# simonamtoft/downsampled-diffusion

Hardware: AMD Instinct MI355X
Metric: images/sec (T=1000 sampling), 256x256 dDDPM-x3 (higher is better)
Workload: dtype f32

## Files before the change

downsampled-diffusion_amd/csrc/conv_wino.hip:

```cpp
#include <atomic>
#include <cstdlib>
#include <type_traits>
#include <utility>

#include "cluster_sync.h"
#include "conv_common.h"
#include "pack_elems.h"

namespace ddk {

__device__ __attribute__((aligned(128))) float g_wino_zero[32];

struct WinoParams {
    const float* src0;
    const float* src1;
    const float* wu;
    const float* bias;
    const float* resid;
    float* out;
    int c0, c1, cin;
    int B, H, W, TH, TW;
    int N, tiles;
    int splits, chunks, chunks_per_split;
    long long slab_stride;
// ... 391 lines not shown
        };
        const float m2 = group_sum((sq4(keep[0][0]) + sq4(keep[0][1])) + (sq4(keep[1][0]) + sq4(keep[1][1])), red + 128);
        if (!CL) {
            if (tid < 16 && (cq & (qpg - 1)) == 0) p.gn_part[(long long)tile_m * p.groups + n0 / p.cpg + gl] = make_float2(mean, m2);
        } else {
            const int image = tile_m / p.cl_np;
            unsigned long long* rec = reinterpret_cast<unsigned long long*>(p.cl_rec) + ((long long)tile_m * gridDim.y + tile_n) * 16;
            unsigned* cnt = p.cl_cnt + ((long long)image * gridDim.y + tile_n) * 16;
            int* gave_up = reinterpret_cast<int*>(red + 256);
            if (tid == 0) *gave_up = 0;
            if (tid < 16 && (cq & (qpg - 1)) == 0) cl_store_stats(rec + gl, mean, m2);
            const int gn = n0 + (tid & 15) * 4;
            float4 ga, be, ts = make_float4(0.f, 0.f, 0.f, 0.f);
            auto load_affine = [&] {
                ga = *reinterpret_cast<const float4*>(p.gn_gamma + gn);
                be = *reinterpret_cast<const float4*>(p.gn_beta + gn);
                if (p.gn_temb) {
                    const int b_img = (int)((long long)t0 / ((long long)p.TH * p.TW));
                    const long long tr = p.gn_temb_rows ? p.gn_temb_rows[b_img] : b_img;
                    ts = *reinterpret_cast<const float4*>(p.gn_temb + tr * p.gn_temb_stride + gn);
                }
            };
            long long oo[2];
            float4 rs[2][2];
#pragma unroll
            for (int it = 0; it < 2; ++it) {
                const int item = tid + it * 512;
                const int t = item >> 5, a = (item >> 4) & 1;
                const int g = t0 + t;
                const unsigned tmp = fdiv_u((unsigned)g, p.dTW);
                const int tx = g - (int)tmp * p.TW;
                const unsigned bq = fdiv_u(tmp, p.dTH);
                const int ty = (int)tmp - (int)bq * p.TH;
                oo[it] = ((((long long)bq * p.H + 2 * ty + a) * p.W) + 2 * tx) * p.N + gn;
            }
            auto load_resid = [&] {
#pragma unroll
                for (int it = 0; it < 2; ++it) {
                    rs[it][0] = rs[it][1] = make_float4(0.f, 0.f, 0.f, 0.f);
                    if (p.resid) {
                        rs[it][0] = *reinterpret_cast<const float4*>(p.resid + oo[it]);
                        rs[it][1] = *reinterpret_cast<const float4*>(p.resid + oo[it] + p.N);
                    }
                }
            };
            if (wid != 0) { load_affine(); load_resid(); }
            if (wid == 0) {
                asm volatile("s_waitcnt vmcnt(0)" ::: "memory");
                if (lane == 0) __hip_atomic_fetch_add(cnt, 1u, __ATOMIC_RELAXED, __HIP_MEMORY_SCOPE_AGENT);
                load_affine();
                load_resid();
                if (lane == 0 && cl_wait_ge<4>(cnt, (unsigned)p.cl_np, p.cl_fail)) *gave_up = 1;
            }
            __syncthreads();
            const unsigned long long* r0 = reinterpret_cast<const unsigned long long*>(p.cl_rec) +
                                           ((long long)image * p.cl_np * gridDim.y + tile_n) * 16 + gl;
            const bool poisoned = *gave_up != 0;
            float rm[8], rq[8];
            cl_load_stats(r0, (long long)gridDim.y * 16, p.cl_np, rm, rq);
            if (tid == 0) cl_depart(cnt, cnt + 1, (unsigned)p.cl_np);
            const float2 st = cl_merge_stats(rm, rq, p.cl_np, 128.0f * (float)p.cpg, p.gn_eps, poisoned);
            const float gmean = st.x, rstd = st.y;
            auto fin = [&](float4 v) {
                return make_float4(mish_f((v.x - gmean) * rstd * ga.x + be.x) + ts.x, mish_f((v.y - gmean) * rstd * ga.y + be.y) + ts.y,
                                   mish_f((v.z - gmean) * rstd * ga.z + be.z) + ts.z, mish_f((v.w - gmean) * rstd * ga.w + be.w) + ts.w);
            };
#pragma unroll
            for (int it = 0; it < 2; ++it) {
                *reinterpret_cast<float4*>(p.out + oo[it]) = f4add(fin(keep[it][0]), rs[it][0]);
                *reinterpret_cast<float4*>(p.out + oo[it] + p.N) = f4add(fin(keep[it][1]), rs[it][1]);
            }
        }
    }
    if (DBG && tid == 0) {
        asm volatile("s_waitcnt vmcnt(0)" ::: "memory");
        const int wg = (blockIdx.x + gridDim.x * (blockIdx.y + gridDim.y * blockIdx.z)) & 1023;
        g_wino_stamps[wg * 8 + 6] = __builtin_amdgcn_s_memrealtime();
        g_wino_stamps[wg * 8 + 7] = 1;
    }
}

#include "conv_wino2_kernel.inc"
#include "conv_winoT_kernel.inc"

enum { WINO_V_OLD = 0, WINO_V_D = 1, WINO_V_F = 2 };
static int wino_variant(int B, int H, int W, int N) {
#ifdef DDK_TUNING
    if (const char* e = getenv("DDK_WINO_VARIANT")) {
        const int v = atoi(e);
        if (v == WINO_V_OLD || v == WINO_V_D || (v == WINO_V_F && N % 128 == 0)) return v;
    }
#endif
    const long long mt = ceil_div((long long)B * (H / 2) * (W / 2), WBT);
    return (N % 128 == 0 && mt * (N / 128) >= 224) ? WINO_V_F : WINO_V_D;
}
static int wino_nt(int variant) { return variant == WINO_V_F ? 128 : WBN; }
bool conv_wino_ok(int kind, int H, int W, int cin, int N) {
    return kind == DDK_CONV3X3_S1 && H >= 2 && W >= 2 && H % 2 == 0 && W % 2 == 0 && cin > 0 && cin % 32 == 0 && N % 64 == 0;
}

int conv_wino_splits(int B, int H, int W, int cin, int N) {
    const long long tiles = (long long)B * (H / 2) * (W / 2);
    const long long wgs = ceil_div(tiles, WBT) * (N / wino_nt(wino_variant(B, H, W, N)));
    const int chunks = cin / 32;
    int s = 1;
    while (wgs * s < 256 && s * 2 <= chunks) s *= 2;
    const int cps = (int)ceil_div(chunks, s);
    return (int)ceil_div(chunks, cps);
}

static int wino_stats_shape_parts(int B, int H, int W, int cin, int N, int groups) {
    if (!conv_wino_ok(DDK_CONV3X3_S1, H, W, cin, N) || groups <= 0 || N % groups) return 0;
    const int cpg = N / groups, tpi = (H / 2) * (W / 2), nt_w = wino_nt(wino_variant(B, H, W, N));
    if (cpg % 4 || nt_w % cpg || nt_w / cpg > 8 || tpi % WBT || tpi / WBT > 32) return 0;
    return tpi / WBT;
}
int conv_wino_stats_parts(int B, int H, int W, int cin, int N, int groups) {
    if (conv_wino_splits(B, H, W, cin, N) != 1) return 0;
    return wino_stats_shape_parts(B, H, W, cin, N, groups);
}

bool convT_wino_ok(int H, int W, int cin, int N) {
    return H >= 2 && W >= 2 && H % 2 == 0 && W % 2 == 0 && cin > 0 && cin % 32 == 0 && N > 0 && N % WT_NT == 0;
}
int convT_wino_splits(int B, int H, int W, int cin, int N) {
    const long long wgs = ceil_div((long long)B * (H / 2) * (W / 2), WBT) * (N / WT_NT) * 4;
    const int chunks = cin / 32;
    int s = 1;
    while (wgs * s < 256 && s * 2 <= chunks) s *= 2;
    const int cps = (int)ceil_div(chunks, s);
    return (int)ceil_div(chunks, cps);
}
int convT_wino_forward(const ddk_conv_args& a, int splits, hipStream_t st) {
    WinoParams p{};
    p.src0 = a.src0; p.wu = a.weight_wino; p.bias = a.bias; p.out = a.out;
    p.c0 = a.c0; p.c1 = 0; p.cin = a.c0;
    p.B = a.B; p.H = a.H; p.W = a.W; p.TH = a.H / 2; p.TW = a.W / 2;
    p.N = a.N; p.tiles = a.B * p.TH * p.TW;
    p.chunks = p.cin / 32;
    p.chunks_per_split = (int)ceil_div(p.chunks, splits);
    p.splits = (int)ceil_div(p.chunks, p.chunks_per_split);
    p.slab_stride = (long long)a.B * (2 * a.H) * (2 * a.W) * a.N;
    p.dTW = make_fastdiv_u((unsigned)p.TW);
    p.dTH = make_fastdiv_u((unsigned)p.TH);
    if (p.splits > 1) p.out = static_cast<float*>(a.workspace);
    dim3 grid((unsigned)ceil_div(p.tiles, WBT), (unsigned)(a.N / WT_NT), (unsigned)(4 * p.splits));
#ifdef DDK_TUNING
    if (getenv("DDK_WINO_STAMPS")) {
        hipLaunchKernelGGL(convT_wino_kernel<1>, grid, dim3(1024), WT_LDS_FL * sizeof(float), st, p);
        return check_launch("convT_wino_kernel<dbg>");
    }
#endif
    hipLaunchKernelGGL(convT_wino_kernel<0>, grid, dim3(1024), WT_LDS_FL * sizeof(float), st, p);
    return check_launch("convT_wino_kernel");
}

int conv_wino_init_device() {
    DDK_HIP(hipFuncSetAttribute(reinterpret_cast<const void*>(&convT_wino_kernel<0>), hipFuncAttributeMaxDynamicSharedMemorySize,
                                (int)(WT_LDS_FL * sizeof(float))));
#ifdef DDK_TUNING
    DDK_HIP(hipFuncSetAttribute(reinterpret_cast<const void*>(&convT_wino_kernel<1>), hipFuncAttributeMaxDynamicSharedMemorySize,
                                (int)(WT_LDS_FL * sizeof(float))));
#endif
    DDK_HIP(hipFuncSetAttribute(reinterpret_cast<const void*>(&conv3x3_wino_kernel<0>), hipFuncAttributeMaxDynamicSharedMemorySize,
                                (int)(W_LDS_FLOATS * sizeof(float))));
    DDK_HIP(hipFuncSetAttribute(reinterpret_cast<const void*>(&conv3x3_wino_kernel<0, true>), hipFuncAttributeMaxDynamicSharedMemorySize,
                                (int)(W_LDS_FLOATS * sizeof(float))));
    DDK_HIP(hipFuncSetAttribute(reinterpret_cast<const void*>(&conv3x3_wino2_kernel<2, 0, false>), hipFuncAttributeMaxDynamicSharedMemorySize,
                                (int)(W2<2>::LDS_FL * sizeof(float))));
    DDK_HIP(hipFuncSetAttribute(reinterpret_cast<const void*>(&conv3x3_wino2_kernel<2, 0, true>), hipFuncAttributeMaxDynamicSharedMemorySize,
                                (int)(W2<2>::LDS_FL * sizeof(float))));
    DDK_HIP(hipFuncSetAttribute(reinterpret_cast<const void*>(&conv3x3_wino2_kernel<4, 0, false>), hipFuncAttributeMaxDynamicSharedMemorySize,
                                (int)(W2<4>::LDS_FL * sizeof(float))));
    DDK_HIP(hipFuncSetAttribute(reinterpret_cast<const void*>(&conv3x3_wino2_kernel<4, 0, true>), hipFuncAttributeMaxDynamicSharedMemorySize,
                                (int)(W2<4>::LDS_FL * sizeof(float))));
#ifdef DDK_TUNING
#define W2_DBG_ATTR(P_, D_) DDK_HIP(hipFuncSetAttribute(reinterpret_cast<const void*>(&conv3x3_wino2_kernel<P_, D_, false>), \
                                                hipFuncAttributeMaxDynamicSharedMemorySize, (int)(W2<P_>::LDS_FL * sizeof(float))))
    W2_DBG_ATTR(2, 1); W2_DBG_ATTR(2, 7); W2_DBG_ATTR(2, 9); W2_DBG_ATTR(2, 15); W2_DBG_ATTR(2, 17);
    W2_DBG_ATTR(4, 1); W2_DBG_ATTR(4, 7); W2_DBG_ATTR(4, 9); W2_DBG_ATTR(4, 15); W2_DBG_ATTR(4, 17);
#undef W2_DBG_ATTR
    DDK_HIP(hipFuncSetAttribute(reinterpret_cast<const void*>(&conv3x3_wino_kernel<1>), hipFuncAttributeMaxDynamicSharedMemorySize, (int)(W_LDS_FLOATS * sizeof(float))));
    DDK_HIP(hipFuncSetAttribute(reinterpret_cast<const void*>(&conv3x3_wino_kernel<2>), hipFuncAttributeMaxDynamicSharedMemorySize, (int)(W_LDS_FLOATS * sizeof(float))));
    DDK_HIP(hipFuncSetAttribute(reinterpret_cast<const void*>(&conv3x3_wino_kernel<3>), hipFuncAttributeMaxDynamicSharedMemorySize, (int)(W_LDS_FLOATS * sizeof(float))));
    DDK_HIP(hipFuncSetAttribute(reinterpret_cast<const void*>(&conv3x3_wino_kernel<4>), hipFuncAttributeMaxDynamicSharedMemorySize, (int)(W_LDS_FLOATS * sizeof(float))));
#endif
    return DDK_OK;
}

int conv_wino_cluster_np(int B, int H, int W, int cin, int N, int groups) {
    const int np = conv_wino_stats_parts(B, H, W, cin, N, groups);
    if (np <= 0 || np > 8) return 0;
    const int nt_w = wino_nt(wino_variant(B, H, W, N));
    if (N / groups > 32 || nt_w % (N / groups)) return 0;
    if (nt_w / (N / groups) > 8) return 0;
    const long long mt = (long long)B * np, nt = N / nt_w;
    if ((mt * nt) % 8) return 0;
    const long long run = mt * nt / 8;
    const long long per_round = run < 32 ? run : 32;
    if (run % (np * nt) || per_round % (np * nt)) return 0;
    return np;
}
int conv_wino_cluster_split_np(int B, int H, int W, int cin, int N, int groups, int* splits_out) {
    if (!conv_wino_ok(DDK_CONV3X3_S1, H, W, cin, N)) return 0;
    const int splits = conv_wino_splits(B, H, W, cin, N);
    if (splits_out) *splits_out = splits;
    if (splits <= 1 || splits > 4) return 0;
    const int np = wino_stats_shape_parts(B, H, W, cin, N, groups);
    if (np <= 0 || np > 8) return 0;
    const int variant = wino_variant(B, H, W, N);
    if (variant != WINO_V_D) return 0;
    const int nt_w = wino_nt(variant);
    if (N / groups > 32 || nt_w % (N / groups) || nt_w / (N / groups) > 8) return 0;
    const long long mt = (long long)B * np, nt = N / nt_w;
    if (mt * nt * splits > 256) return 0;
    return np;
}
size_t conv_wino_cluster_pair_words(int B, int H, int W, int N) {
    return (size_t)ceil_div((long long)B * (H / 2) * (W / 2), WBT) * (size_t)(N / WBN) * 16;
}
size_t conv_wino_cluster_ws_floats(int B, int H, int W, int N) {
    const long long mt = (long long)B * (H / 2) * (W / 2) / WBT, nt = N / WBN;
    return (size_t)(mt * nt * 32 + (long long)B * nt * 16);
}

bool conv_wino_cluster_device_ok() {
    static std::atomic<int> cached[64];
    int dev = 0;
    if (hipGetDevice(&dev) != hipSuccess || dev < 0 || dev >= 64) return false;
    int v = cached[dev].load(std::memory_order_relaxed);
    if (v == 0) {
        int cus = 0, xccs = 0;
        bool ok = hipDeviceGetAttribute(&cus, hipDeviceAttributeMultiprocessorCount, dev) == hipSuccess && cus == 256;
        ok = ok && hipDeviceGetAttribute(&xccs, hipDeviceAttributeNumberOfXccs, dev) == hipSuccess && xccs == 8;
        ok = ok && !getenv("HSA_CU_MASK") && !getenv("ROC_GLOBAL_CU_MASK");
        (void)hipGetLastError();
        v = ok ? 1 : 2;
        cached[dev].store(v, std::memory_order_relaxed);
    }
    return v == 1;
// ... 60 lines not shown
    if (v == D_) {                                                                                                     \
        if (f) hipLaunchKernelGGL((conv3x3_wino2_kernel<2, D_, false>), grid2, dim3(768), lds, st, p);                 \
        else hipLaunchKernelGGL((conv3x3_wino2_kernel<4, D_, false>), grid2, dim3(768), lds, st, p);                   \
        return check_launch("conv3x3_wino2_kernel<dbg>");                                                              \
    }
            W2_DBG_LAUNCH(7) W2_DBG_LAUNCH(9) W2_DBG_LAUNCH(15) W2_DBG_LAUNCH(17)
#undef W2_DBG_LAUNCH
            if (f) hipLaunchKernelGGL((conv3x3_wino2_kernel<2, 1, false>), grid2, dim3(768), lds, st, p);
            else hipLaunchKernelGGL((conv3x3_wino2_kernel<4, 1, false>), grid2, dim3(768), lds, st, p);
            return check_launch("conv3x3_wino2_kernel<dbg>");
        }
#endif
        if (fuse) {
            if (f) hipLaunchKernelGGL((conv3x3_wino2_kernel<2, 0, true>), grid2, dim3(768), lds, st, p);
            else hipLaunchKernelGGL((conv3x3_wino2_kernel<4, 0, true>), grid2, dim3(768), lds, st, p);
            return check_launch("conv3x3_wino2_kernel<cluster>");
        }
        if (f) hipLaunchKernelGGL((conv3x3_wino2_kernel<2, 0, false>), grid2, dim3(768), lds, st, p);
        else hipLaunchKernelGGL((conv3x3_wino2_kernel<4, 0, false>), grid2, dim3(768), lds, st, p);
        return check_launch("conv3x3_wino2_kernel");
    }
    dim3 grid((unsigned)ceil_div(p.tiles, WBT), (unsigned)(a.N / WBN), (unsigned)p.splits);
#ifdef DDK_TUNING
    if (getenv("DDK_WINO_STAMPS")) {
        const int v = getenv("DDK_WINO_DEBUG") ? atoi(getenv("DDK_WINO_DEBUG")) : 1;
        if (v == 2) hipLaunchKernelGGL(conv3x3_wino_kernel<2>, grid, dim3(512), W_LDS_FLOATS * sizeof(float), st, p);
        else if (v == 3) hipLaunchKernelGGL(conv3x3_wino_kernel<3>, grid, dim3(512), W_LDS_FLOATS * sizeof(float), st, p);
        else if (v == 4) hipLaunchKernelGGL(conv3x3_wino_kernel<4>, grid, dim3(512), W_LDS_FLOATS * sizeof(float), st, p);
        else hipLaunchKernelGGL(conv3x3_wino_kernel<1>, grid, dim3(512), W_LDS_FLOATS * sizeof(float), st, p);
        return check_launch("conv3x3_wino_kernel<dbg>");
    }
#endif
    if (fuse) {
        hipLaunchKernelGGL((conv3x3_wino_kernel<0, true>), grid, dim3(512), W_LDS_FLOATS * sizeof(float), st, p);
        return check_launch("conv3x3_wino_kernel<cluster>");
    }
    hipLaunchKernelGGL(conv3x3_wino_kernel<0>, grid, dim3(512), W_LDS_FLOATS * sizeof(float), st, p);
    return check_launch("conv3x3_wino_kernel");
}

__global__ __launch_bounds__(256) void occupy_kernel(unsigned long long ticks, unsigned* sink) {
    extern __shared__ float occupy_lds[];
    occupy_lds[threadIdx.x] = (float)threadIdx.x;
    __syncthreads();
    const unsigned long long t_begin = __builtin_amdgcn_s_memrealtime();
    while (__builtin_amdgcn_s_memrealtime() - t_begin < ticks) __builtin_amdgcn_s_sleep(32);
    if (occupy_lds[(threadIdx.x + 1) & 255] < 0.f && sink) *sink = 1;
}

unsigned conv_wino_cluster_timeouts() { return cl_timeouts_read(); }

int cluster_fail_check(unsigned* word, hipStream_t st, const char* who, const char* tail) {
    unsigned v = 0;
    DDK_HIP(hipMemcpyAsync(&v, word, sizeof(v), hipMemcpyDeviceToHost, st));
    DDK_HIP(hipStreamSynchronize(st));
    if (v == 0) return DDK_OK;
    DDK_HIP(hipMemsetAsync(word, 0, sizeof(v), st));
    set_error("%s: %u workgroup(s) gave up waiting for their cluster%s", who, v, tail);
    return DDK_ERR_CLUSTER;
}

}

extern "C" int ddk_pack_conv_weight_wino(const float* w_oihw, float* dst, int O, int I, int i_pad, ddk_stream_t s) {
    using namespace ddk;
    DDK_REQUIRE(w_oihw && dst && O > 0 && I > 0 && i_pad >= I && i_pad % 32 == 0, "pack_conv_weight_wino: arguments (i_pad % 32 == 0)");
    const long long total = (long long)O * i_pad;
    DDK_REQUIRE(total < (1LL << 31), "pack_conv_weight_wino: 2^31 (n, c) pairs or more");
    const long long blocks = ceil_div(total, 256);
    hipLaunchKernelGGL(pack_conv_weight_wino_kernel<false>, dim3((unsigned)(blocks < 4096 ? blocks : 4096)), dim3(256), 0, as_stream(s), w_oihw,
                       dst, O, I, i_pad, total, 0, I);
    return check_launch("pack_conv_weight_wino_kernel");
}

extern "C" int ddk_pack_convT_weight_wino(const float* w_iohw, float* dst, int I, int O, int i_pad, ddk_stream_t s) {
    using namespace ddk;
    DDK_REQUIRE(w_iohw && dst && O > 0 && I > 0 && i_pad >= I && i_pad % 32 == 0, "pack_convT_weight_wino: arguments (i_pad % 32 == 0)");
    const long long total = (long long)O * i_pad;
    const long long blocks = ceil_div(total, 256);
    hipLaunchKernelGGL(pack_convT_weight_wino_kernel, dim3((unsigned)(blocks < 4096 ? blocks : 4096)), dim3(256), 0, as_stream(s), w_iohw, dst,
                       I, O, i_pad, total);
    return check_launch("pack_convT_weight_wino_kernel");
}
extern "C" int ddk_convT_wino_splits(int B, int H, int W, int cin, int N) {
    if (!ddk::convT_wino_ok(H, W, cin, N)) return 0;
    return ddk::convT_wino_splits(B, H, W, cin, N);
}

extern "C" int ddk_pack_conv_weight_wino_dgrad(const float* w_oihw, float* dst, int O, int I, int c_lo, int c_hi, int o_pad, ddk_stream_t s) {
    using namespace ddk;
    DDK_REQUIRE(w_oihw && dst && O > 0 && I > 0 && c_lo >= 0 && c_hi > c_lo && c_hi <= I && o_pad >= O && o_pad % 32 == 0,
                "pack_conv_weight_wino_dgrad: arguments (0 <= c_lo < c_hi <= I, o_pad % 32 == 0)");
    const long long total = (long long)(c_hi - c_lo) * o_pad;
    DDK_REQUIRE(total < (1LL << 31), "pack_conv_weight_wino_dgrad: 2^31 (n, c) pairs or more");
    const long long blocks = ceil_div(total, 256);
    hipLaunchKernelGGL(pack_conv_weight_wino_kernel<true>, dim3((unsigned)(blocks < 4096 ? blocks : 4096)), dim3(256), 0, as_stream(s), w_oihw,
                       dst, c_hi - c_lo, O, o_pad, total, c_lo, I);
    return check_launch("pack_conv_weight_wino_kernel<dgrad>");
}

#ifdef DDK_TUNING
extern "C" int ddk_debug_read_wino_timeline(unsigned long long* host_out) {
    if (hipDeviceSynchronize() != hipSuccess) return -2;
    return hipMemcpyFromSymbol(host_out, HIP_SYMBOL(ddk::g_wino_timeline), sizeof(unsigned long long) * 12 * 8 * 2) == hipSuccess ? 0 : -2;
}
extern "C" int ddk_debug_read_wino_stamps(unsigned long long* host_out) {
    if (hipDeviceSynchronize() != hipSuccess) return -2;
    if (hipMemcpyFromSymbol(host_out, HIP_SYMBOL(ddk::g_wino_stamps), sizeof(unsigned long long) * 8 * 1024) != hipSuccess) return -2;
    static unsigned long long zeros[8 * 1024];
    return hipMemcpyToSymbol(HIP_SYMBOL(ddk::g_wino_stamps), zeros, sizeof(zeros)) == hipSuccess ? 0 : -2;
}
#endif

extern "C" int ddk_conv_gn_partials(int B, int H, int W, int cin, int N, int groups) {
    return ddk::conv_wino_stats_parts(B, H, W, cin, N, groups);
}

extern "C" int ddk_conv_wino_splits(int B, int H, int W, int cin, int N) {
    if (!ddk::conv_wino_ok(DDK_CONV3X3_S1, H, W, cin, N)) return 0;
    return ddk::conv_wino_splits(B, H, W, cin, N);
}

extern "C" int ddk_conv3x3_gn_mish_cluster_ok(int B, int H, int W, int cin, int N, int groups) {
    if (!ddk::conv_wino_cluster_device_ok()) return 0;
    const int np = ddk::conv_wino_cluster_np(B, H, W, cin, N, groups);
    return np > 0 ? np : ddk::conv_wino_cluster_split_np(B, H, W, cin, N, groups, nullptr);
}
extern "C" size_t ddk_conv3x3_gn_mish_cluster_workspace_bytes(int B, int H, int W, int N) {
    if (B <= 0 || H <= 0 || W <= 0 || N <= 0 || N % ddk::WBN) return 0;
    return ((size_t)B * 8 * 16 + 16 + ddk::conv_wino_cluster_ws_floats(B, H, W, N)) * sizeof(float);
}
extern "C" size_t ddk_conv3x3_gn_mish_cluster_split_workspace_bytes(int B, int H, int W, int cin, int N, int groups) {
    int splits = 1;
    if (ddk::conv_wino_cluster_split_np(B, H, W, cin, N, groups, &splits) <= 0) return 0;
    return ddk_conv3x3_gn_mish_cluster_workspace_bytes(B, H, W, N) +
           (ddk::conv_wino_cluster_pair_words(B, H, W, N) + (size_t)(splits - 1) * B * H * W * N) * sizeof(float);
}
extern "C" int ddk_conv3x3_gn_mish_cluster_check(void* workspace, int B, ddk_stream_t s) {
    using namespace ddk;
    DDK_REQUIRE(workspace && B > 0, "conv3x3_gn_mish_cluster_check: arguments");
    return cluster_fail_check(cl_words(static_cast<float*>(workspace), B).fail, as_stream(s), "conv3x3_gn_mish_cluster",
                              "; the output is invalid (NaN tiles)");
}

extern "C" int ddk_debug_occupy(int workgroups, int lds_bytes, int microseconds, ddk_stream_t s) {
    using namespace ddk;
    DDK_REQUIRE(workgroups > 0 && workgroups <= 4096 && lds_bytes >= 1024 && lds_bytes <= 160 * 1024 && microseconds > 0 &&
                    microseconds <= 200000, "debug_occupy: 1..4096 workgroups, 1 KiB..160 KiB of LDS, at most 0.2 s");
    DDK_HIP(hipFuncSetAttribute(reinterpret_cast<const void*>(&occupy_kernel), hipFuncAttributeMaxDynamicSharedMemorySize, lds_bytes));
    hipLaunchKernelGGL(occupy_kernel, dim3((unsigned)workgroups), dim3(256), (size_t)lds_bytes, as_stream(s),
                       (unsigned long long)microseconds * 100ull, static_cast<unsigned*>(nullptr));
    return check_launch("occupy_kernel");
}

extern "C" int ddk_conv3x3_gn_mish_cluster(const float* src0, int c0, const float* src1, int c1, const float* weight_wino, const float* bias,
                                           const float* gamma, const float* beta, const float* temb, int temb_stride, const float* addend,
                                           float* out, int B, int H, int W, int N, int groups, float eps, void* workspace,
                                           size_t workspace_bytes, ddk_stream_t s) {
    using namespace ddk;
    DDK_REQUIRE(src0 && weight_wino && gamma && beta && out && workspace, "conv3x3_gn_mish_cluster: null pointer");
    DDK_REQUIRE(conv_wino_cluster_device_ok() && ddk_conv3x3_gn_mish_cluster_ok(B, H, W, c0 + c1, N, groups) > 0,
                "conv3x3_gn_mish_cluster: shape or device not eligible (ddk_conv3x3_gn_mish_cluster_ok)");
    const size_t plain_bytes = ddk_conv3x3_gn_mish_cluster_workspace_bytes(B, H, W, N);
    const size_t split_bytes = ddk_conv3x3_gn_mish_cluster_split_workspace_bytes(B, H, W, c0 + c1, N, groups);
    DDK_REQUIRE(workspace_bytes >= (split_bytes ? split_bytes : plain_bytes) && aligned16(workspace), "conv3x3_gn_mish_cluster: workspace");
    float* ws = static_cast<float*>(workspace);
// ... 23 lines not shown
```

downsampled-diffusion_amd/csrc/ddk_internal.h:

```cpp
#pragma once
#include <hip/hip_runtime.h>

#include <cstdarg>
#include <cstdint>
#include <cstdio>

#include "ddk.h"

#ifdef DDK_HOST_SANITIZE
#include "host_sanitize.h"
#endif

namespace ddk {

void set_error(const char* fmt, ...);

inline int fail_arg(const char* what) {
    set_error("bad argument: %s", what);
    return DDK_ERR_ARG;
}

inline int check_launch(const char* what) {
    hipError_t e = hipGetLastError();
    if (e != hipSuccess) {
// ... 51 lines not shown

__device__ __forceinline__ float wave_sum(float v) {
#pragma unroll
    for (int o = 32; o > 0; o >>= 1) v += __shfl_xor(v, o, 64);
    return v;
}

__device__ __forceinline__ float wave_max(float v) {
#pragma unroll
    for (int o = 32; o > 0; o >>= 1) v = fmaxf(v, __shfl_xor(v, o, 64));
    return v;
}

__device__ __forceinline__ float block_sum(float v, float* red) {
    v = wave_sum(v);
    const int lane = threadIdx.x & 63, wid = threadIdx.x >> 6, nw = blockDim.x >> 6;
    __syncthreads();
    if (lane == 0) red[wid] = v;
    __syncthreads();
    float t = (lane < nw) ? red[lane] : 0.0f;
    t = wave_sum(t);
    return t;
}

__device__ __forceinline__ float block_max(float v, float* red) {
    v = wave_max(v);
    const int lane = threadIdx.x & 63, wid = threadIdx.x >> 6, nw = blockDim.x >> 6;
    __syncthreads();
    if (lane == 0) red[wid] = v;
    __syncthreads();
    float t = (lane < nw) ? red[lane] : -INFINITY;
    t = wave_max(t);
    return t;
}

int ensure_device_init();
int conv_init_device();
int wgrad_init_device();

size_t conv_workspace_bytes(int kind, int B, int H, int W, int cin, int N);
struct ConvLnFold {
    const float* c1;
    const float* c2;
    float eps;
};
struct WinoGnFuse {
    const float* gamma;
    const float* beta;
    const float* temb;
    const long long* temb_rows;
    int temb_stride;
    float eps;
    int groups;
    float* records;
    unsigned* counters;
    unsigned* fail;
    unsigned* pairs = nullptr;
    const float* res_x = nullptr;
    const float* res_w = nullptr;
    const float* res_b = nullptr;
    int res_cin = 0, res_ld = 0;
};
bool conv_ln_fold_ok(int B, int H, int W, int cin, int N);
int conv_forward(const ddk_conv_args& a, hipStream_t st, const ConvLnFold* ln = nullptr, const WinoGnFuse* fuse = nullptr);
int conv_splits(int kind, int B, int H, int W, int cin, int N);
bool conv_wino_ok(int kind, int H, int W, int cin, int N);
int conv_wino_splits(int B, int H, int W, int cin, int N);
int conv_wino_forward(const ddk_conv_args& a, int splits, hipStream_t st, const WinoGnFuse* fuse = nullptr);
int conv_wino_cluster_np(int B, int H, int W, int cin, int N, int groups);
int conv_wino_cluster_split_np(int B, int H, int W, int cin, int N, int groups, int* splits_out);
size_t conv_wino_cluster_pair_words(int B, int H, int W, int N);
bool conv_wino_variant_new(int B, int H, int W, int N);
bool conv_wino_cluster_device_ok();
size_t conv_wino_cluster_ws_floats(int B, int H, int W, int N);
unsigned conv_wino_cluster_timeouts();
unsigned conv_first_cluster_timeouts();
unsigned level_chain_cluster_timeouts();
struct ClWords { unsigned* counters; unsigned* fail; };
inline ClWords cl_words(float* cl, int B) { return {reinterpret_cast<unsigned*>(cl), reinterpret_cast<unsigned*>(cl + (size_t)B * 8 * 16)}; }
int cluster_fail_check(unsigned* word, hipStream_t st, const char* who, const char* tail);
bool convT_wino_ok(int H, int W, int cin, int N);
int convT_wino_splits(int B, int H, int W, int cin, int N);
int convT_wino_forward(const ddk_conv_args& a, int splits, hipStream_t st);
int conv_wino_init_device();
int conv_wino_stats_parts(int B, int H, int W, int cin, int N, int groups);
bool conv_first_ok(int cin, int N, int H, int W, int groups);
int conv_first(const float* x, const float* wp, const float* bias, float* out, float* gn_partials, int B, int H, int W, int cin, int N,
               int groups, int64_t* counter, int64_t* t_cur, hipStream_t st);
int conv_first_init_device();
bool conv_first_gn_ok(int cin, int N, int H, int W, int groups);
size_t conv_first_gn_ws_floats(int B, int H, int W);
int conv_first_gn(const float* x, const float* wp, const float* bias, const float* gamma, const float* beta, const float* temb,
                  int temb_stride, const long long* temb_rows, float eps, float* out, int B, int H, int W, int cin, int N, int groups,
                  float* records, unsigned* counters, unsigned* fail, int64_t* counter, int64_t* t_cur, hipStream_t st);
bool conv1x1_sm_ok(long long M, int c0, int c1, int N);
int conv1x1_sm(const float* src0, int c0, const float* src1, int c1, const float* w, const float* bias, const float* resid, float* out,
               long long M, int N, const ConvLnFold* ln, hipStream_t st);
int conv1x1_sm_init_device();
bool conv1x1_stream_ok(long long M, int cin, int N);
int conv1x1_stream(const float* x, int cin, const float* w, const float* bias, const float* dmish_src, const float* resid, float* out,
                   float* mish_out, long long M, int N, int pre_mish, int post_mish, hipStream_t st);
bool conv1x1_ws_ok(long long M, int K, int N);
int conv1x1_ws(const float* x, const float* w, const float* bias, const float* resid, float* out, long long M, int N, const ConvLnFold* ln,
               hipStream_t st, int images = 0);
int conv1x1_ws_init_device();
struct AddendSlabs {
    int n = 1;
    long long stride = 0;
    const float* bias = nullptr;
};
bool conv_gn_local_ok(int H, int W, int cin, int c0, int N, int groups);
int conv_gn_local(const float* src0, int c0, const float* src1, int c1, const float* w, const float* bias, const float* gamma,
                  const float* beta, const float* temb, int temb_stride, const long long* temb_rows, const float* addend, float* out,
                  int B, int H, int W, int N, int groups, float eps, hipStream_t st, const AddendSlabs& as = AddendSlabs(),
                  const AddendSlabs& src_slabs = AddendSlabs());
int conv_gn_local_init_device();
bool conv_gn_wlocal_ok(int H, int W, int cin, int c0, int N, int groups);
int conv_gn_wlocal(const float* src0, int c0, const float* src1, int c1, const float* w, const float* bias, const float* gamma,
                   const float* beta, const float* temb, int temb_stride, const long long* temb_rows, const float* addend, float* out,
                   int B, int H, int W, int N, int groups, float eps, hipStream_t st, const AddendSlabs& as = AddendSlabs(),
                   const AddendSlabs& src_slabs = AddendSlabs());
double conv_flops(int kind, int B, int H, int W, int cin, int N);
size_t groupnorm_workspace_bytes(int B, int HW, int C, int groups);
int gn_train_nsplit(int HW, int cpg);
int gn_stats_partials(const float* x, float* part, int B, int HW, int C, int groups, int ns, hipStream_t st);
int groupnorm_mish(const float* x, const float* gamma, const float* beta, const float* temb, int temb_stride,
                   const float* addend, float* out, int B, int HW, int C, int groups, float eps, void* ws, size_t ws_bytes,
                   hipStream_t st, const long long* temb_rows = nullptr);
int groupnorm_mish_ex(const float* x, int nslab, long long slab_stride, const float* cbias, const float* gamma,
                      const float* beta, const float* temb, int temb_stride, const float* addend, float* out, int B, int HW, int C,
                      int groups, float eps, void* ws, size_t ws_bytes, hipStream_t st, const long long* temb_rows = nullptr);
int groupnorm_mish_parts(const float* x, const float* part, int np, const float* gamma, const float* beta, const float* temb,
                         int temb_stride, const float* addend, float* out, int B, int HW, int C, int groups, float eps, hipStream_t st,
                         const long long* temb_rows = nullptr, const float* rc_x = nullptr, const float* rc_w = nullptr,
                         const float* rc_b = nullptr, int rc_cin = 0, int rc_ld = 0);
int chan_layernorm(const float* x, const float* g, const float* b, float* out, long long M, int C, float eps, hipStream_t st);
int groupnorm_mish_generic(const float* x, const float* gamma, const float* beta, const float* temb, int temb_stride, const float* addend,
                           float* out, int B, int HW, int CP, int C, int groups, float eps, hipStream_t st, const long long* temb_rows = nullptr);
int chan_layernorm_generic(const float* x, const float* g, const float* b, float* out, long long M, int CP, int C, float eps, hipStream_t st);
int unary(int op, const float* x, float* out, long long n, hipStream_t st);
int add(const float* a, const float* b, float* out, long long n, hipStream_t st);
int avgpool2(const float* x, float* out, int B, int H, int W, int C, hipStream_t st);
int upsample_nearest2(const float* x, float* out, int B, int H, int W, int C, hipStream_t st);
size_t linattn_context_workspace_bytes(int B, int HW, int heads);
int linattn_context(const float* qkv, float* ctx, int B, int HW, int heads, void* workspace, size_t workspace_bytes, hipStream_t st,
                    bool kv_only = false);
bool attn_fold_ok(int C, int heads);
bool attn_kvctx_ok(int B, int HW, int C, int heads);
size_t attn_kvctx_workspace_bytes(int B, int HW);
int attn_kvctx(const float* x, const float* w_kv, const float* c1, const float* c2, float ln_eps, float* ctx, int B, int HW, void* workspace,
               size_t workspace_bytes, hipStream_t st);
size_t attn_fold_out_floats(int B);
int attn_fold(const float* ctx, const float* wqg, const float* c1q, const float* c2q, const float* wout, const float* bout, float* A,
              float* a1, float* a2, int B, int C, int heads, hipStream_t st);
int linattn_apply(const float* qkv, const float* ctx, float* out, int B, int HW, int heads, hipStream_t st);
int linattn_fused_small(const float* qkv, float* ctx, float* out, int B, int HW, int heads, hipStream_t st);
bool linattn_small_qkv_ok(int HW, int C);
int linattn_small_qkv_init_device();
int qkv_operand_pack(const float* lnw, float* wop, int heads, int cp, hipStream_t st);
int linattn_small_qkv(const float* x, const float* wop, const float* c1, const float* c2, float ln_eps, float* ctx, float* out, int B, int HW,
                      int C, int heads, hipStream_t st);
int time_mlp(const int64_t* t, const float* freqs, const float* w1t, const float* b1, const float* w2t, const float* b2,
             float* act, float* raw, int B, int dim, hipStream_t st);
int time_proj(const float* act, const float* wt, const float* bias, float* out, int B, int dim, int n_out, hipStream_t st);
int conv1x1_small_n(const float* x, const float* w, const float* bias, float* out, long long M, int C, int n_out, hipStream_t st);
struct InpaintOps {
// ... 75 lines not shown
```

downsampled-diffusion_amd/csrc/unet_plan.hip:

```cpp
#include <algorithm>
#include <mutex>
#include <string>
#include <vector>

#include "ddk_internal.h"
#include "level_chain.h"

namespace ddk {

constexpr int HEADS = 4;
constexpr int HIDDEN = HEADS * 32;
constexpr int GROUPS = 8;
constexpr float GN_EPS = 1e-5f, LN_EPS = 1e-5f;

static inline int pad32(int c) { return (c + 31) / 32 * 32; }

enum PackKind { PK_COPY = 0, PK_CONV = 1, PK_CONVT = 2, PK_LINEAR_T = 3, PK_WINO = 4, PK_LOCAL = 5, PK_WLOCAL = 6, PK_FIRST = 7, PK_CONVT_WINO = 8,
                PK_ROWS = 9 , PK_LOCAL1 = 10 ,
                PK_CONVT_LOCAL = 11  };

struct Slot {
    std::string name;
    long long numel;
    int kind;
    size_t off;
    int O, I, KH, KW, i_pad, ld, col0;
    int split = 0, split_pad = 0;
    int attn = -1;
};

struct ConvW {
    size_t w = 0, b = 0;
    bool has_bias = false;
    int cin = 0, cin_pad = 0, cout = 0;
    size_t wu = 0;
    bool has_wu = false;
    size_t wl = 0;
    bool has_wl = false;
    size_t wwl = 0;
    bool has_wwl = false;
    size_t wf = 0;
    bool has_wf = false;
    size_t wl1 = 0;
    bool has_wl1 = false;
    size_t wtl = 0;
    bool has_wtl = false;
};
struct NormW { size_t g = 0, b = 0; int c_real = 0; };
struct ResW {
    int ci = 0, ci_pad = 0, co = 0, temb_off = 0, ci_real = 0, co_real = 0;
    ConvW c1, c2, res;
    NormW n1, n2;
    bool has_res = false;
};
struct AttnW {
    int c = 0, c_real = 0;
    NormW ln;
    ConvW qkv, out;
    size_t qkv_lnw = 0, ln_c1 = 0, ln_c2 = 0;
    size_t qkv_op = 0;
};

}

using namespace ddk;

struct ChainKey {
    StepKind kind;
    const void* bufs[12];
    const void* ws;
    const void* noise;
    int B, H, W, t_start, device;
    unsigned long long pack_epoch;
    bool operator==(const ChainKey& o) const {
        for (int i = 0; i < 12; ++i)
            if (bufs[i] != o.bufs[i]) return false;
        return kind == o.kind && ws == o.ws && noise == o.noise && B == o.B && H == o.H && W == o.W && t_start == o.t_start &&
               device == o.device && pack_epoch == o.pack_epoch;
    }
};
struct SamplerGraph {
    ChainKey key;
    hipGraph_t graph = nullptr;
    hipGraphExec_t exec = nullptr;
    hipGraph_t graph_multi = nullptr;
    hipGraphExec_t exec_multi = nullptr;
    hipEvent_t done = nullptr;
    unsigned long long last_use = 0;
};
constexpr int SAMPLER_MULTI = 16;

struct ddk_unet {
    std::mutex mu;
    std::vector<SamplerGraph> graphs;
    unsigned long long use_clock = 0;
    unsigned long long pack_epoch = 0;
    struct {
        const void* ws = nullptr;
        int t_start = -1, B = 0, H = 0, W = 0;
        unsigned long long pack_epoch = 0;
        std::vector<int64_t> map;
    } table;
    ddk_unet_config cfg;
    int cluster_gn = 1;
    int cluster_limit = 1 << 30;
    int cluster_np_max = 8;
    bool cluster_split = true;
    bool attn_kvctx = true;
    bool fold_down_reduce = false;
    bool first_gn = true;
    int level_chain = 9;
    int level_chain_max_batch = 32;
    int attn_fold_min_hw = 256;
    bool attn_fold = true;
    bool generic = false;
    std::vector<int> dimp;
    std::vector<Slot> slots;
    size_t packed_floats = 0;
    int L = 0;
    std::vector<int> dims;
    int time_dim = 0, temb_total = 0;
    size_t freqs = 0, w1t = 0, b1 = 0, w2t = 0, b2 = 0, temb_wt = 0, temb_bias = 0;
    std::vector<ResW> down_res, up_res;
    std::vector<AttnW> down_attn, up_attn;
    std::vector<ConvW> down_conv, up_conv;
    ResW mid1, mid2;
    AttnW mid_attn;
    ConvW final_conv;
    NormW final_norm;
    size_t final_w = 0, final_b = 0;

    size_t alloc(size_t n) {
        const size_t o = packed_floats;
        packed_floats += (n + 3) / 4 * 4;
        return o;
    }
    size_t add_copy(const std::string& name, long long n) {
        const size_t o = alloc((size_t)n);
        slots.push_back(Slot{name, n, PK_COPY, o, 0, 0, 0, 0, 0, 0, 0});
        return o;
    }
    void add_copy_at(const std::string& name, long long n, size_t off) {
        slots.push_back(Slot{name, n, PK_COPY, off, 0, 0, 0, 0, 0, 0, 0});
    }
    ConvW add_conv(const std::string& prefix, int cout, int cin, int k, bool bias, bool gn_follows = false, int split = 0, bool local = false) {
        ConvW c;
        c.cin = cin; c.cin_pad = split > 0 ? pad32(split) + pad32(cin - split) : pad32(cin); c.cout = cout;
        const int cout_rows = pad32(cout);
        c.w = alloc((size_t)cout_rows * k * k * c.cin_pad);
        Slot sl{prefix + "weight", (long long)cout * cin * k * k, PK_CONV, c.w, cout, cin, k, k, c.cin_pad, 0, 0};
        if (split > 0 && c.cin_pad != cin) { sl.split = split; sl.split_pad = pad32(split); }
        slots.push_back(sl);
        c.has_bias = bias;
        if (bias) {
            c.b = alloc((size_t)cout_rows);
            slots.push_back(Slot{prefix + "bias", cout, PK_COPY, c.b, 0, 0, 0, 0, 0, 0, 0});
        }
        if (generic) return c;
        if (k == 1 && bias && cout % 32 == 0 && c.cin_pad == cin && cin % 32 == 0) {
            c.wl1 = alloc((size_t)cout * c.cin_pad);
            c.has_wl1 = true;
            slots.push_back(Slot{prefix + "weight", (long long)cout * cin, PK_LOCAL1, c.wl1, cout, cin, 1, 1, c.cin_pad, 0, 0});
        }
        if (k == 3 && cout % 64 == 0) {
            c.wu = alloc((size_t)16 * cout * c.cin_pad);
            c.has_wu = true;
            slots.push_back(Slot{prefix + "weight", (long long)cout * cin * k * k, PK_WINO, c.wu, cout, cin, k, k, c.cin_pad, 0, 0});
        }
        if (k == 3 && (gn_follows || local) && cout % 32 == 0) {
            c.wl = alloc((size_t)9 * cout * c.cin_pad);
            c.has_wl = true;
            slots.push_back(Slot{prefix + "weight", (long long)cout * cin * k * k, PK_LOCAL, c.wl, cout, cin, k, k, c.cin_pad, 0, 0});
            if (gn_follows && (c.cin_pad <= 320 || c.cin_pad == 512)) {
                c.wwl = alloc((size_t)16 * cout * c.cin_pad);
                c.has_wwl = true;
                slots.push_back(Slot{prefix + "weight", (long long)cout * cin * k * k, PK_WLOCAL, c.wwl, cout, cin, k, k, c.cin_pad, 0, 0});
            }
        }
        return c;
    }
    ConvW add_convT(const std::string& prefix, int ch, bool local = false) {
        ConvW c;
        c.cin = ch; c.cin_pad = pad32(ch); c.cout = ch;
        c.w = alloc((size_t)16 * pad32(ch) * pad32(ch));
        slots.push_back(Slot{prefix + "weight", (long long)16 * ch * ch, PK_CONVT, c.w, ch, ch, 4, 4, pad32(ch), 0, 0});
        c.has_bias = true;
        c.b = alloc((size_t)pad32(ch));
        slots.push_back(Slot{prefix + "bias", ch, PK_COPY, c.b, 0, 0, 0, 0, 0, 0, 0});
        if (local && ch % 32 == 0 && !generic) {
            c.wtl = alloc((size_t)16 * ch * ch);
            c.has_wtl = true;
            slots.push_back(Slot{prefix + "weight", (long long)16 * ch * ch, PK_CONVT_LOCAL, c.wtl, ch, ch, 4, 4, ch, 0, 0});
// ... 38 lines not shown
        a.c = generic ? pad32(c) : c;
        a.c_real = c;
        const size_t s0 = slots.size();
        a.qkv = add_conv(p + "fn.fn.to_qkv.", 3 * HIDDEN, c, 1, false);
        const size_t s1 = slots.size();
        a.out = add_conv(p + "fn.fn.to_out.", c, HIDDEN, 1, true);
        const size_t s2 = slots.size();
        a.ln = add_norm(p + "fn.norm.g", p + "fn.norm.b", c);
        for (size_t i = s0; i < s1; ++i) slots[i].attn = n_attn;
        for (size_t i = s2; i < slots.size(); ++i) slots[i].attn = n_attn;
        a.qkv_lnw = alloc((size_t)3 * HIDDEN * pad32(c));
        a.ln_c1 = alloc((size_t)3 * HIDDEN);
        a.ln_c2 = alloc((size_t)3 * HIDDEN);
        a.qkv_op = alloc((size_t)3 * HIDDEN * pad32(c));
        attn_all.push_back(a);
        ++n_attn;
        return a;
    }
};

static int total_temb(const ddk_unet& u) {
    int tot = 0;
    for (int l = 0; l < u.L; ++l) tot += 2 * u.dims[l + 1];
    tot += 2 * u.dims[u.L];
    for (int i = 0; i < u.L - 1; ++i) tot += 2 * u.dims[u.L - 1 - i];
    return tot;
}

extern "C" ddk_unet* ddk_unet_create(const ddk_unet_config* cfg) {
    if (!cfg || cfg->n_levels < 1 || cfg->n_levels > 8 || cfg->in_ch < 1 || cfg->chan < 8 || cfg->chan % 8 ||
        cfg->chan > 512) {
        set_error("unet_create: need 1 <= n_levels <= 8, in_ch >= 1, unet_chan a multiple of 8 in [8, 512]");
        return nullptr;
    }
    for (int i = 0; i < cfg->n_levels; ++i)
        if (cfg->mults[i] < 1) { set_error("unet_create: unet_dims entries must be >= 1"); return nullptr; }
    if (cfg->mults[0] != 1) {
        set_error("unet_create: unet_dims[0] must be 1 (the reference's final Block(dim, dim) meets dim * unet_dims[0] channels "
                  "otherwise and raises, unet.py:69-72)");
        return nullptr;
    }
    {
        int ndev = 0;
        if (hipGetDeviceCount(&ndev) == hipSuccess && ndev > 0 && ensure_device_init() != DDK_OK) return nullptr;
        (void)hipGetLastError();
    }
    ddk_unet* u = new ddk_unet();
    u->cfg = *cfg;
    u->L = cfg->n_levels;
    u->generic = cfg->chan % 32 != 0;
    for (int i = 0; i < cfg->n_levels; ++i)
        if (cfg->chan * cfg->mults[i] > 512) { set_error("unet_create: level widths above 512 channels are not supported"); delete u; return nullptr; }
    u->dims.push_back(cfg->in_ch);
    for (int i = 0; i < u->L; ++i) u->dims.push_back(cfg->chan * cfg->mults[i]);
    for (int d : u->dims) u->dimp.push_back(u->generic ? pad32(d) : d);
    u->time_dim = cfg->chan;
    u->temb_total = total_temb(*u);
    const int td = u->time_dim;

    u->freqs = u->add_copy("@sinusoidal_freqs", td / 2);
    u->w1t = u->alloc((size_t)td * 4 * td);
    u->slots.push_back(Slot{"time_mlp.1.weight", (long long)4 * td * td, PK_LINEAR_T, u->w1t, 4 * td, td, 0, 0, 0, 4 * td, 0});
    u->b1 = u->add_copy("time_mlp.1.bias", 4 * td);
    u->w2t = u->alloc((size_t)4 * td * td);
    u->slots.push_back(Slot{"time_mlp.3.weight", (long long)4 * td * td, PK_LINEAR_T, u->w2t, td, 4 * td, 0, 0, 0, td, 0});
    u->b2 = u->add_copy("time_mlp.3.bias", td);
    u->temb_wt = u->alloc((size_t)td * u->temb_total);
    u->temb_bias = u->alloc((size_t)u->temb_total);

    int cur = 0;
    for (int l = 0; l < u->L; ++l) {
        const std::string p = "downs." + std::to_string(l) + ".";
        const int ci = u->dims[l], co = u->dims[l + 1];
        u->down_res.push_back(u->add_res(p + "0.", ci, co, cur));
        if (l == 0 && ci <= 8 && co <= 256 && !u->generic) {
            ConvW& c1 = u->down_res[0].c1;
            const int K2 = (9 * ci + 1) / 2;
            c1.wf = u->alloc((size_t)(co / 32) * K2 * 64);
            c1.has_wf = true;
            u->slots.push_back(Slot{p + "0.block1.block.0.weight", (long long)co * ci * 9, PK_FIRST, c1.wf, co, ci, 3, 3, 0, 0, 0});
        }
        u->down_res.push_back(u->add_res(p + "1.", co, co, cur));
        u->down_attn.push_back(u->add_attn(p + "2.", co));
        if (l < u->L - 1) u->down_conv.push_back(u->add_conv(p + "3.conv.", co, co, 3, true, false, 0, l == u->L - 2));
    }
    const int mid = u->dims[u->L];
    u->mid1 = u->add_res("mid_block1.", mid, mid, cur);
    u->mid_attn = u->add_attn("mid_attn.", mid);
    u->mid2 = u->add_res("mid_block2.", mid, mid, cur);
    for (int i = 0; i < u->L - 1; ++i) {
        const std::string p = "ups." + std::to_string(i) + ".";
        const int din = u->dims[u->L - 1 - i], dout = u->dims[u->L - i];
        u->up_res.push_back(u->add_res(p + "0.", 2 * dout, din, cur, dout));
        u->up_res.push_back(u->add_res(p + "1.", din, din, cur));
        u->up_attn.push_back(u->add_attn(p + "2.", din));
        u->up_conv.push_back(u->add_convT(p + "3.conv.", din, i == 0));
    }
    u->final_conv = u->add_conv("final_conv.0.block.0.", cfg->chan, cfg->chan, 3, true, true);
    u->final_norm = u->add_norm("final_conv.0.block.1.weight", "final_conv.0.block.1.bias", cfg->chan);
    if (u->generic) {
        u->final_w = u->alloc((size_t)cfg->in_ch * pad32(cfg->chan));
        u->slots.push_back(Slot{"final_conv.1.weight", (long long)cfg->in_ch * cfg->chan, PK_ROWS, u->final_w, cfg->in_ch, cfg->chan, 0, 0, 0,
                                pad32(cfg->chan), 0});
    } else {
        u->final_w = u->add_copy("final_conv.1.weight", (long long)cfg->in_ch * cfg->chan);
    }
    u->final_b = u->add_copy("final_conv.1.bias", cfg->in_ch);
    if (cur != u->temb_total) {
        set_error("unet_create: internal temb accounting mismatch");
        delete u;
        return nullptr;
    }
    return u;
}

static void drop_graphs(ddk_unet* u) {
    for (SamplerGraph& g : u->graphs) {
        if (g.exec) (void)hipGraphExecDestroy(g.exec);
        if (g.graph) (void)hipGraphDestroy(g.graph);
        if (g.exec_multi) (void)hipGraphExecDestroy(g.exec_multi);
        if (g.graph_multi) (void)hipGraphDestroy(g.graph_multi);
        if (g.done) (void)hipEventDestroy(g.done);
    }
    u->graphs.clear();
    u->table.ws = nullptr;
}

extern "C" void ddk_unet_destroy(ddk_unet* u) {
    if (!u) return;
    if (!u->graphs.empty()) (void)hipDeviceSynchronize();
    drop_graphs(u);
    delete u;
}

extern "C" int ddk_sampler_invalidate(ddk_unet* u) {
    DDK_REQUIRE(u, "sampler_invalidate: null plan");
    std::lock_guard<std::mutex> lock(u->mu);
    if (!u->graphs.empty()) DDK_HIP(hipDeviceSynchronize());
    drop_graphs(u);
    return DDK_OK;
}
static void destroy_entry(SamplerGraph& g) {
    if (g.done) { (void)hipEventSynchronize(g.done); (void)hipEventDestroy(g.done); }
    if (g.exec) (void)hipGraphExecDestroy(g.exec);
    if (g.graph) (void)hipGraphDestroy(g.graph);
    if (g.exec_multi) (void)hipGraphExecDestroy(g.exec_multi);
    if (g.graph_multi) (void)hipGraphDestroy(g.graph_multi);
}

extern "C" int ddk_sampler_release_workspace(ddk_unet* u, const void* workspace) {
    DDK_REQUIRE(u && workspace, "sampler_release_workspace: arguments");
    std::lock_guard<std::mutex> lock(u->mu);
    for (size_t i = 0; i < u->graphs.size();) {
        if (u->graphs[i].key.ws == workspace) {
            destroy_entry(u->graphs[i]);
            u->graphs.erase(u->graphs.begin() + (long)i);
        } else {
            ++i;
        }
    }
    if (u->table.ws == workspace) u->table.ws = nullptr;
    return DDK_OK;
}

extern "C" int ddk_unet_set_option(ddk_unet* u, int option, int value) {
    DDK_REQUIRE(u, "unet_set_option: null plan");
    static const struct {
        int option;
        bool drops_graphs;
        void (*set)(ddk_unet&, int);
    } options[] = {
        {DDK_OPT_CLUSTER_GROUPNORM, true, [](ddk_unet& p, int v) { p.cluster_gn = v < 0 ? 0 : v > 2 ? 2 : v; }},
        {DDK_OPT_ATTENTION_FOLD, true, [](ddk_unet& p, int v) { p.attn_fold = v != 0; }},
        {DDK_OPT_ATTENTION_KV_CONTEXT, true, [](ddk_unet& p, int v) { p.attn_kvctx = v != 0; }},
        {DDK_OPT_FIRST_GROUPNORM, true, [](ddk_unet& p, int v) { p.first_gn = v != 0; }},
        {DDK_OPT_LEVEL_CHAIN, true, [](ddk_unet& p, int v) {
             p.level_chain = v == 1 ? 9 : v == 2 ? 1 : v == 3 ? 15 : v == 4 ? 6 : v == 8 ? 2 : v == 16 ? 4 : v != 0 ? 9 : 0;
         }},
        {DDK_OPT_FOLD_DOWNSAMPLE_REDUCE, true, [](ddk_unet& p, int v) { p.fold_down_reduce = v != 0; }},
        {10, true, [](ddk_unet& p, int v) { p.level_chain_max_batch = v; }},
        {9, true, [](ddk_unet& p, int v) { p.attn_fold_min_hw = v; }},
        {2, false, [](ddk_unet& p, int v) { p.cluster_limit = v; }},
        {4, true, [](ddk_unet& p, int v) { p.cluster_np_max = v; }},
        {11, true, [](ddk_unet& p, int v) { p.cluster_split = v != 0; }},
    };
    for (const auto& o : options) {
        if (o.option != option) continue;
        std::lock_guard<std::mutex> lock(u->mu);
        if (o.drops_graphs) {
            if (!u->graphs.empty()) DDK_HIP(hipDeviceSynchronize());
            drop_graphs(u);
        }
        o.set(*u, value);
        return DDK_OK;
    }
    return fail_arg("unet_set_option: unknown option");
}
extern "C" unsigned ddk_debug_cluster_timeouts(void) {
    unsigned sum = 0;
    for (unsigned v : {ddk::conv_wino_cluster_timeouts(), ddk::conv_first_cluster_timeouts(), ddk::level_chain_cluster_timeouts()}) {
        if (v == ~0u) return ~0u;
        sum += v;
    }
    return sum;
}
extern "C" int ddk_unet_num_slots(const ddk_unet* u) { return u ? (int)u->slots.size() : 0; }
extern "C" const char* ddk_unet_slot_name(const ddk_unet* u, int slot) {
    return (u && slot >= 0 && slot < (int)u->slots.size()) ? u->slots[slot].name.c_str() : nullptr;
}
extern "C" long long ddk_unet_slot_numel(const ddk_unet* u, int slot) {
    return (u && slot >= 0 && slot < (int)u->slots.size()) ? u->slots[slot].numel : -1;
}
extern "C" size_t ddk_unet_packed_bytes(const ddk_unet* u) { return u ? u->packed_floats * sizeof(float) : 0; }

__global__ __launch_bounds__(64) void ln_fold_kernel(const float* __restrict__ w, const float* __restrict__ g, const float* __restrict__ b,
                                                     float* __restrict__ wg, float* __restrict__ c1, float* __restrict__ c2, int C, int cp) {
    const int n = blockIdx.x;
    float s1 = 0.f, s2 = 0.f;
    for (int c = threadIdx.x; c < cp; c += 64) {
        const float wv = w[(long long)n * cp + c];
        const float gv = c < C ? g[c] : 0.f, bv = c < C ? b[c] : 0.f;
        wg[(long long)n * cp + c] = wv * gv;
        s1 += wv * gv;
        s2 += wv * bv;
    }
    s1 = wave_sum(s1);
    s2 = wave_sum(s2);
    if (threadIdx.x == 0) { c1[n] = s1; c2[n] = s2; }
}

static int fold_attn(const AttnW& a, float* P, hipStream_t st) {
    hipLaunchKernelGGL(ln_fold_kernel, dim3(3 * HIDDEN), dim3(64), 0, st, P + a.qkv.w, P + a.ln.g, P + a.ln.b, P + a.qkv_lnw, P + a.ln_c1,
                       P + a.ln_c2, a.c, pad32(a.c));
    DDK_TRY(check_launch("ln_fold_kernel"));
    return qkv_operand_pack(P + a.qkv_lnw, P + a.qkv_op, HEADS, pad32(a.c), st);
}

static void weights_changed(const ddk_unet* u) {
    ddk_unet* m = const_cast<ddk_unet*>(u);
    std::lock_guard<std::mutex> lock(m->mu);
    ++m->pack_epoch;
}

extern "C" int ddk_unet_finalize_pack(const ddk_unet* u, void* packed, ddk_stream_t s) {
    DDK_REQUIRE(u && packed, "unet_finalize_pack: arguments");
    weights_changed(u);
    for (const AttnW& a : u->attn_all) DDK_TRY(fold_attn(a, static_cast<float*>(packed), as_stream(s)));
    return DDK_OK;
}

extern "C" int ddk_unet_pack_slot(const ddk_unet* u, int slot, const float* canonical, void* packed, ddk_stream_t s) {
    DDK_REQUIRE(u && canonical && packed && slot >= 0 && slot < (int)u->slots.size(), "unet_pack_slot: arguments");
    const Slot& sl = u->slots[slot];
    float* dst = static_cast<float*>(packed) + sl.off;
    weights_changed(u);
    int rc;
    switch (sl.kind) {
        case PK_COPY:
            DDK_HIP(hipMemcpyAsync(dst, canonical, (size_t)sl.numel * sizeof(float), hipMemcpyDeviceToDevice, as_stream(s)));
            rc = DDK_OK;
            break;
        case PK_CONV:
            rc = sl.split > 0 ? ddk_pack_conv_weight_split(canonical, dst, sl.O, sl.I, sl.KH, sl.KW, sl.i_pad, sl.split, sl.split_pad, s)
                              : ddk_pack_conv_weight(canonical, dst, sl.O, sl.I, sl.KH, sl.KW, sl.i_pad, s);
            break;
        case PK_CONVT: rc = sl.i_pad == sl.I ? ddk_pack_convT_weight(canonical, dst, sl.I, sl.O, s)
                                             : ddk_pack_convT_weight_padded(canonical, dst, sl.I, sl.O, sl.i_pad, s); break;
        case PK_ROWS:
            DDK_HIP(hipMemcpy2DAsync(dst, (size_t)sl.ld * sizeof(float), canonical, (size_t)sl.I * sizeof(float), (size_t)sl.I * sizeof(float),
                                     (size_t)sl.O, hipMemcpyDeviceToDevice, as_stream(s)));
            rc = DDK_OK;
            break;
        case PK_LINEAR_T: rc = ddk_pack_linear_T(canonical, dst, sl.O, sl.I, sl.ld, sl.col0, s); break;
        case PK_WINO: rc = ddk_pack_conv_weight_wino(canonical, dst, sl.O, sl.I, sl.i_pad, s); break;
        case PK_LOCAL: rc = ddk_pack_conv_weight_local(canonical, dst, sl.O, sl.I, sl.i_pad, s); break;
        case PK_LOCAL1: rc = ddk_pack_conv1x1_weight_local(canonical, dst, sl.O, sl.I, sl.i_pad, s); break;
        case PK_CONVT_LOCAL: rc = ddk_pack_convT_weight_local(canonical, dst, sl.I, sl.O, s); break;
        case PK_WLOCAL: rc = ddk_pack_conv_weight_wino_local(canonical, dst, sl.O, sl.I, sl.i_pad, s); break;
        case PK_FIRST: rc = ddk_pack_conv_weight_first(canonical, dst, sl.O, sl.I, s); break;
        case PK_CONVT_WINO: rc = ddk_pack_convT_weight_wino(canonical, dst, sl.I, sl.O, sl.i_pad, s); break;
        default: return fail_arg("unet_pack_slot: slot kind");
    }
    DDK_TRY(rc);
    if (sl.attn >= 0) DDK_TRY(fold_attn(u->attn_all[sl.attn], static_cast<float*>(packed), as_stream(s)));
    return DDK_OK;
}

namespace ddk {

struct Layout {
    size_t act = 0;
    size_t qkv = 0, o = 0, ctx = 0, splitk = 0, gn_ws = 0, cl = 0, chain = 0;
    std::vector<size_t> skip;
    size_t xpad = 0, temb = 0, tact = 0;
    size_t off_A = 0, off_B = 0, off_C = 0, off_raw = 0, off_a1 = 0, off_res = 0, off_xn = 0, off_qkv = 0, off_o = 0, off_ctx = 0,
           off_splitk = 0, off_gn = 0, off_xpad = 0, off_temb = 0, off_tact = 0, off_cl = 0, off_chain = 0;
    std::vector<size_t> off_skip;
    size_t total = 0;
};

static size_t al4(size_t n) { return (n + 3) / 4 * 4; }

static void upd(size_t& m, size_t v) { if (v > m) m = v; }

static bool convT_wino_use(int B, int H, int W, int cin, int N) {
    return convT_wino_ok(H, W, cin, N) && convT_wino_splits(B, H, W, cin, N) <= 2;
}
static bool use_wino(const ConvW& cw, int H, int W, int cin, int N) {
    return cw.has_wu && conv_wino_ok(DDK_CONV3X3_S1, H, W, cin, N);
}
static int conv3_splits(const ConvW& cw, int B, int H, int W, int cin, int N) {
    return use_wino(cw, H, W, cin, N) ? conv_wino_splits(B, H, W, cin, N) : conv_splits(DDK_CONV3X3_S1, B, H, W, cin, N);
}
static size_t conv3_ws_floats(const ConvW& cw, int B, int H, int W, int cin, int N) {
    if (!use_wino(cw, H, W, cin, N)) return conv_workspace_bytes(DDK_CONV3X3_S1, B, H, W, cin, N) / 4;
    const int s = conv_wino_splits(B, H, W, cin, N);
    return s > 1 ? (size_t)s * B * H * W * N : 0;
}

constexpr size_t CL_PAIR_WORDS = 128 * 16;
static size_t cl_counter_floats(int B) { return (size_t)B * 8 * 16 + 16 + (size_t)B * 64 + CL_PAIR_WORDS; }
static size_t cl_chain_offset(int B) { return (size_t)B * 8 * 16 + 16; }
static size_t cl_pair_offset(int B) { return (size_t)B * 8 * 16 + 16 + (size_t)B * 64; }
constexpr int CHAIN_BUFS = 18;
constexpr int CHAIN8_BUFS = 5;

static void res_sizes(const ResW& r, int B, int H, int W, Layout& ly) {
    const size_t M = (size_t)B * H * W;
    upd(ly.act, M * r.co);
    upd(ly.splitk, conv3_ws_floats(r.c1, B, H, W, r.ci_pad, r.co));
    upd(ly.splitk, conv3_ws_floats(r.c2, B, H, W, r.co, r.co));
    if (r.has_res) upd(ly.splitk, conv_workspace_bytes(DDK_CONV1X1, B, H, W, r.ci_pad, r.co) / 4);
    upd(ly.gn_ws, groupnorm_workspace_bytes(B, H * W, r.co, GROUPS) / 4);
    upd(ly.gn_ws, (size_t)2 * GROUPS * (M / 128 + 1));
    upd(ly.cl, cl_counter_floats(B) + conv_wino_cluster_ws_floats(B, H, W, r.co));
    if (H * W % 128 == 0 && H * W / 128 <= 8) upd(ly.cl, cl_counter_floats(B) + conv_first_gn_ws_floats(B, H, W));
}

static void attn_sizes(const AttnW& a, int B, int H, int W, Layout& ly) {
    const size_t M = (size_t)B * H * W;
    upd(ly.act, M * a.c);
    upd(ly.qkv, M * 3 * HIDDEN);
    upd(ly.o, M * HIDDEN);
    upd(ly.ctx, (size_t)B * HEADS * 32 * 32);
    upd(ly.splitk, linattn_context_workspace_bytes(B, H * W, HEADS) / 4);
    if (attn_kvctx_ok(B, H * W, a.c, HEADS)) upd(ly.splitk, attn_kvctx_workspace_bytes(B, H * W) / 4);
    upd(ly.splitk, conv_workspace_bytes(DDK_CONV1X1, B, H, W, a.c, 3 * HIDDEN) / 4);
    upd(ly.splitk, conv_workspace_bytes(DDK_CONV1X1, B, H, W, HIDDEN, a.c) / 4);
}

static bool chain_plain(const ResW& r, bool wino) {
    return r.ci == 256 && r.co == 256 && !r.has_res && r.c1.has_bias && r.c2.has_bias && (wino ? r.c1.has_wwl && r.c2.has_wwl : r.c1.has_wl && r.c2.has_wl);
}
static bool chain_att(const AttnW& a) { return a.c == 256 && a.out.has_wl1 && a.out.has_bias; }
static bool chain_cat(const ResW& r, bool wino) {
    return r.ci == 512 && r.ci_pad == 512 && r.co == 256 && r.has_res && r.res.has_wl1 && r.res.has_bias && r.c1.cin_pad == 512 && r.c1.has_bias &&
           r.c2.has_bias && (wino ? r.c1.has_wwl && r.c2.has_wwl : r.c1.has_wl && r.c2.has_wl);
}
static bool level_chain_shape_ok(const ddk_unet& u, int H0, int W0) {
    if (u.generic || u.L < 2) return false;
    const int sh = u.L - 1;
    if ((H0 >> sh) != 4 || (W0 >> sh) != 4 || (H0 & ((1 << sh) - 1)) || (W0 & ((1 << sh) - 1))) return false;
    if (u.dimp[u.L] != 256 || u.dimp[u.L - 1] != 256 || GROUPS != 8) return false;
    return chain_plain(u.down_res[2 * sh], false) && chain_plain(u.down_res[2 * sh + 1], false) && chain_plain(u.mid1, false) &&
           chain_plain(u.mid2, false) && chain_plain(u.up_res[1], false) && chain_att(u.down_attn[sh]) && chain_att(u.mid_attn) &&
           chain_att(u.up_attn[0]) && chain_cat(u.up_res[0], false);
}
static bool level8_chain_shape_ok(const ddk_unet& u, int H0, int W0) {
    if (u.generic || u.L < 3) return false;
    const int sh = u.L - 2;
    if ((H0 >> sh) != 8 || (W0 >> sh) != 8 || (H0 & ((1 << sh) - 1)) || (W0 & ((1 << sh) - 1))) return false;
    if (u.dimp[sh + 1] != 256 || u.dimp[sh] != 256 || u.dimp[sh + 2] != 256 || GROUPS != 8) return false;
    return chain_plain(u.down_res[2 * sh], true) && chain_plain(u.down_res[2 * sh + 1], true) && chain_att(u.down_attn[sh]) &&
           chain_cat(u.up_res[2], true) && chain_plain(u.up_res[3], true) && chain_att(u.up_attn[1]);
}

static Layout make_layout(const ddk_unet& u, int B, int H0, int W0) {
    Layout ly;
    int H = H0, W = W0;
    ly.skip.resize(u.L);
    for (int l = 0; l < u.L; ++l) {
        res_sizes(u.down_res[2 * l], B, H, W, ly);
        res_sizes(u.down_res[2 * l + 1], B, H, W, ly);
        attn_sizes(u.down_attn[l], B, H, W, ly);
        ly.skip[l] = al4((size_t)B * H * W * u.dimp[l + 1]);
        if (l < u.L - 1) {
            upd(ly.splitk, conv_workspace_bytes(DDK_CONV3X3_S2, B, H, W, u.dimp[l + 1], u.dimp[l + 1]) / 4);
            H /= 2; W /= 2;
            upd(ly.act, (size_t)B * H * W * u.dimp[l + 1]);
// ... 459 lines not shown
    Ctx c{u, P, ws, ly, B, st, temb_table ? temb_table : temb, temb_table ? reinterpret_cast<const long long*>(t) : nullptr};
    if (!fast0) { c.x_first = x; c.x_padded = xpad; }
    c.allow_cluster = allow_cluster;
    float* bufA = ws + ly.off_A;
    float* bufB = ws + ly.off_B;
    float* bufC = ws + ly.off_C;
    float* raw = ws + ly.off_raw;
    float* a1 = ws + ly.off_a1;
    float* gnp = ws + ly.off_gn;

    int H = H0, W = W0;
    const float* cur = xpad;
    int cur_c = pad32(u.cfg.in_ch);
    AddendSlabs cur_ss;
    const bool first_fused = fast0 && c.allow_cluster && u.first_gn && conv_wino_cluster_device_ok() &&
                             conv_first_gn_ok(u.down_res[0].ci, u.down_res[0].co, H0, W0, GROUPS) && u.cluster_limit > 0;
    int64_t* dec_counter = (first_fused && step) ? step->state : nullptr;
    const bool chained = level_chain_use(c, H0, W0);
    const bool chain_edges = chained && (u.level_chain & 8) && u.L >= 2 && u.down_conv[u.L - 2].has_wl && u.down_conv[u.L - 2].has_bias &&
                             u.up_conv[0].has_wtl && u.up_conv[0].cin == 256 && u.down_conv[u.L - 2].cin == 256;
    const bool chained8 = level8_chain_use(c, H0, W0, 2);
    const bool chained8u = level8_chain_use(c, H0, W0, 4);
    for (int l = 0; l < u.L; ++l) {
        float* skip = ws + ly.off_skip[l];
        const int co = u.dimp[l + 1];
        if (chained && l == u.L - 1) {
            DDK_TRY(run_level_chain(c, 0, cur, skip, bufB, chain_edges ? ws + ly.off_skip[l - 1] : nullptr, chain_edges ? bufA : nullptr));
            cur_c = co;
            break;
        }
        const bool level_chained = chained8 && l == u.L - 2 && cur_ss.n == 1;
        if (level_chained) {
            DDK_TRY(run_level_chain(c, 1, cur, skip, nullptr));
        } else if (l == 0 && fast0) {
            const ResW& r = u.down_res[0];
            if (first_fused) {
                float* cl = ws + ly.off_cl;
                const ClWords w = cl_words(cl, B);
                DDK_TRY(conv_first_gn(x, P + r.c1.wf, r.c1.has_bias ? P + r.c1.b : nullptr, P + r.n1.g, P + r.n1.b, c.temb + r.temb_off,
                                      u.temb_total, c.temb_rows, GN_EPS, a1, B, H, W, r.ci, r.co, GROUPS, cl + cl_counter_floats(B),
                                      w.counters, w.fail,
                                      step ? step->state : nullptr, step ? t : nullptr, st));
            } else {
                DDK_TRY(conv_first(x, P + r.c1.wf, r.c1.has_bias ? P + r.c1.b : nullptr, raw, gnp, B, H, W, r.ci, r.co, GROUPS,
                                   step ? step->state : nullptr, step ? t : nullptr, st));
                DDK_TRY(groupnorm_mish_parts(raw, gnp, H * W / 128, P + r.n1.g, P + r.n1.b, c.temb + r.temb_off, u.temb_total, nullptr, a1, B,
                                             H * W, r.co, GROUPS, GN_EPS, st, c.temb_rows));
            }
            ddk_conv_args a{};
            a.kind = DDK_CONV3X3_S1;
            a.src0 = a1; a.c0 = r.co;
            a.weight = P + r.c2.w;
            a.weight_wino = P + r.c2.wu;
            a.bias = r.c2.has_bias ? P + r.c2.b : nullptr;
            a.B = B; a.H = H; a.W = W; a.N = r.co;
            const int cl_np = c.allow_cluster && conv_wino_cluster_device_ok() && r.ci <= 8 ? conv_wino_cluster_np(B, H, W, r.co, r.co, GROUPS) : 0;
            if (cl_np > 0 && cl_np <= u.cluster_np_max && conv_wino_variant_new(B, H, W, r.co) && c.n_cluster++ < u.cluster_limit) {
                a.out = bufB;
                float* cl = ws + ly.off_cl;
                const ClWords w = cl_words(cl, B);
                WinoGnFuse f{P + r.n2.g, P + r.n2.b, nullptr, nullptr, u.temb_total, GN_EPS, GROUPS, cl + cl_counter_floats(B), w.counters, w.fail};
                f.res_x = x; f.res_w = P + r.res.w; f.res_b = r.res.has_bias ? P + r.res.b : nullptr; f.res_cin = r.ci; f.res_ld = r.res.cin_pad;
                DDK_TRY(conv_forward(a, st, nullptr, &f));
            } else {
                a.out = raw;
                a.gn_partials = gnp;
                a.gn_groups = GROUPS;
                DDK_TRY(conv_forward(a, st));
                DDK_TRY(groupnorm_mish_parts(raw, gnp, conv_wino_stats_parts(B, H, W, r.co, r.co, GROUPS), P + r.n2.g, P + r.n2.b, nullptr,
                                             u.temb_total, nullptr, bufB, B, H * W, r.co, GROUPS, GN_EPS, st, nullptr, x, P + r.res.w,
                                             r.res.has_bias ? P + r.res.b : nullptr, r.ci, r.res.cin_pad));
            }
        } else {
            DDK_TRY(run_res(c, u.down_res[2 * l], cur, cur_c, nullptr, 0, bufB, H, W, cur_ss));
            cur_ss = AddendSlabs();
        }
        if (!level_chained) {
            DDK_TRY(run_res(c, u.down_res[2 * l + 1], bufB, co, nullptr, 0, bufC, H, W));
            DDK_TRY(run_attn(c, u.down_attn[l], bufC, skip, H, W));
        }
        if (l < u.L - 1 && chain_edges && l + 1 == u.L - 1) {
            H /= 2; W /= 2;
            cur = skip;
        } else if (l < u.L - 1) {
            const int s2 = conv_splits(DDK_CONV3X3_S2, B, H, W, co, co);
            if (u.fold_down_reduce && s2 > 1 && !(chained && l + 1 == u.L - 1) && !(chained8 && l + 1 == u.L - 2) &&
                res_takes_slab_source(u, u.down_res[2 * l + 2], B, H / 2, W / 2, co)) {
                ddk_conv_args a{};
                a.kind = DDK_CONV3X3_S2;
                a.src0 = skip; a.c0 = co;
                a.weight = P + u.down_conv[l].w;
                a.out = bufA;
                a.B = B; a.H = H; a.W = W; a.N = co;
                a.defer_reduce = 1;
                a.workspace = ws + ly.off_splitk;
                a.workspace_bytes = ly.splitk * sizeof(float);
                DDK_TRY(conv_forward(a, st));
                cur_ss.n = s2;
                cur_ss.stride = (long long)B * (H / 2) * (W / 2) * co;
                cur_ss.bias = u.down_conv[l].has_bias ? P + u.down_conv[l].b : nullptr;
                H /= 2; W /= 2;
                cur = ws + ly.off_splitk;
            } else {
                DDK_TRY(run_conv(c, DDK_CONV3X3_S2, u.down_conv[l], skip, co, nullptr, 0, nullptr, bufA, H, W, co));
                H /= 2; W /= 2;
                cur = bufA;
            }
        } else {
            cur = skip;
        }
        cur_c = co;
    }
    if (!chained) {
        DDK_TRY(run_res(c, u.mid1, cur, cur_c, nullptr, 0, bufB, H, W));
        DDK_TRY(run_attn(c, u.mid_attn, bufB, bufC, H, W));
        DDK_TRY(run_res(c, u.mid2, bufC, cur_c, nullptr, 0, bufA, H, W));
        cur = bufA;
    }
    for (int i = 0; i < u.L - 1; ++i) {
        const int lvl = u.L - 1 - i;
        const float* skip = ws + ly.off_skip[lvl];
        const int dout = u.dimp[lvl + 1], din = u.dimp[lvl];
        if (chained8u && i == 1) {
            DDK_TRY(run_level_chain(c, 2, cur, const_cast<float*>(skip), bufB));
        } else if (!(chained && i == 0)) {
            DDK_TRY(run_res(c, u.up_res[2 * i], cur, cur_c, skip, dout, bufB, H, W));
            DDK_TRY(run_res(c, u.up_res[2 * i + 1], bufB, din, nullptr, 0, bufC, H, W));
            DDK_TRY(run_attn(c, u.up_attn[i], bufC, bufB, H, W));
        }
        if (!(chain_edges && i == 0))
            DDK_TRY(run_conv(c, DDK_CONVT4X4_S2, u.up_conv[i], bufB, din, nullptr, 0, nullptr, bufA, H, W, din));
        H *= 2; W *= 2;
        cur = bufA;
        cur_c = din;
    }
    const int chan = u.generic ? pad32(u.cfg.chan) : u.cfg.chan, n_out = u.cfg.in_ch;
    StepRule plain{};
    plain.kind = StepKind::Eps;
    plain.eps_out = out;
    const StepRule& rule = step ? step->rule : plain;
    ChainHooks hooks{};
    if (step) {
        hooks.chain_state = step->state;
        hooks.dec_counter = dec_counter;
    }
    const int npf = fused_tail_parts(u, B, H, W, cur_c, rule.kind);
    if (npf > 0 && (!step || step->per == (long long)H * W * n_out)) {
        ddk_conv_args a{};
        a.kind = DDK_CONV3X3_S1;
        a.src0 = cur; a.c0 = cur_c;
        a.weight = P + u.final_conv.w;
        a.weight_wino = P + u.final_conv.wu;
        a.bias = u.final_conv.has_bias ? P + u.final_conv.b : nullptr;
        a.out = raw;
        a.B = B; a.H = H; a.W = W; a.N = chan;
        a.gn_partials = gnp;
        a.gn_groups = GROUPS;
        DDK_TRY(conv_forward(a, st));
        const TailIn in{raw, gnp, npf, P + u.final_norm.g, P + u.final_norm.b, GN_EPS, P + u.final_w, P + u.final_b, n_out, B, H * W, chan, GROUPS};
        return final_tail(in, rule, t, hooks, st);
    }
    DDK_TRY(run_conv_gn(c, u.final_conv, cur, cur_c, nullptr, 0, raw, u.final_norm, nullptr, nullptr, a1, H, W, chan));
    float* eps_hat = step ? step->eps_hat : out;
    DDK_TRY(conv1x1_small_n(a1, P + u.final_w, P + u.final_b, eps_hat, (long long)B * H * W, chan, n_out, st));
    return step ? p_update(rule, eps_hat, t, B, step->per, hooks, st) : DDK_OK;
}
// ... 32 lines not shown
        set_error("unet_forward: workspace too small (%zu < %zu)", workspace_bytes, ly.total * sizeof(float));
        return DDK_ERR_WORKSPACE;
    }
    float* ws = static_cast<float*>(workspace);
    DDK_TRY(ensure_device_init());
    DDK_HIP(hipMemsetAsync(ws + ly.off_cl, 0, cl_counter_floats(B) * sizeof(float), as_stream(s)));
    return forward_core(*u, static_cast<const float*>(packed), x, const_cast<int64_t*>(t), out, B, H, W, ws, ly, as_stream(s),
                        u->cluster_gn >= 2);
}

extern "C" int ddk_unet_cluster_check(const ddk_unet* u, void* workspace, int B, int H, int W, ddk_stream_t s) {
    DDK_TRY(check_shape(u, B, H, W));
    DDK_REQUIRE(workspace, "unet_cluster_check: null workspace");
    const Layout ly = make_layout(*u, B, H, W);
    return cluster_fail_check(cl_words(static_cast<float*>(workspace) + ly.off_cl, B).fail, as_stream(s), "in-launch GroupNorm",
                              " (the GPU is shared, masked or partitioned); results on this workspace are invalid -- rerun with "
                              "DDK_OPT_CLUSTER_GROUPNORM = 0");
}

extern "C" double ddk_unet_flops(const ddk_unet* u, int B, int H0, int W0) {
    if (check_shape(u, B, H0, W0) != DDK_OK) return 0;
    double f = 0;
    auto res = [&](const ResW& r, int H, int W) {
        f += conv_flops(DDK_CONV3X3_S1, B, H, W, r.ci_real, r.co_real) + conv_flops(DDK_CONV3X3_S1, B, H, W, r.co_real, r.co_real);
        if (r.has_res) f += conv_flops(DDK_CONV1X1, B, H, W, r.ci_real, r.co_real);
        f += 2.0 * B * u->time_dim * r.co_real;
    };
    auto attn = [&](const AttnW& a, int H, int W) {
        f += conv_flops(DDK_CONV1X1, B, H, W, a.c_real, 3 * HIDDEN) + conv_flops(DDK_CONV1X1, B, H, W, HIDDEN, a.c_real);
        f += 2.0 * 2.0 * B * HEADS * 32.0 * 32.0 * H * W;
    };
    int H = H0, W = W0;
    f += 2.0 * B * (u->time_dim * 4.0 * u->time_dim) * 2;
    for (int l = 0; l < u->L; ++l) {
        res(u->down_res[2 * l], H, W); res(u->down_res[2 * l + 1], H, W); attn(u->down_attn[l], H, W);
        if (l < u->L - 1) { f += conv_flops(DDK_CONV3X3_S2, B, H, W, u->dims[l + 1], u->dims[l + 1]); H /= 2; W /= 2; }
    }
    res(u->mid1, H, W); attn(u->mid_attn, H, W); res(u->mid2, H, W);
    for (int i = 0; i < u->L - 1; ++i) {
        res(u->up_res[2 * i], H, W); res(u->up_res[2 * i + 1], H, W); attn(u->up_attn[i], H, W);
        f += conv_flops(DDK_CONVT4X4_S2, B, H, W, u->up_conv[i].cin, u->up_conv[i].cout);
        H *= 2; W *= 2;
    }
    f += conv_flops(DDK_CONV3X3_S1, B, H, W, u->cfg.chan, u->cfg.chan) + conv_flops(DDK_CONV1X1, B, H, W, u->cfg.chan, u->cfg.in_ch);
    return f;
}

extern "C" double ddk_unet_flops_executed(const ddk_unet* u, int B, int H0, int W0) {
    if (check_shape(u, B, H0, W0) != DDK_OK) return 0;
    double f = 0;
    auto conv3 = [&](const ConvW& cw, int H, int W, int c0, int c1, int N, bool gn) {
        const int cin = c0 + c1;
        if (gn && cw.has_wl && (H * W == 16 || (H * W == 4 && B % 4 == 0)) && conv_gn_local_ok(H, W, cin, c0, N, GROUPS))
            return 2.0 * B * H * W * 9.0 * cin * N;
        if (gn && cw.has_wwl && H * W == 64 && conv_gn_wlocal_ok(H, W, cin, c0, N, GROUPS)) return 2.0 * B * (H * W / 4) * 16.0 * cin * N;
        if (use_wino(cw, H, W, cin, N)) return 2.0 * (double)(ceil_div((long long)B * (H / 2) * (W / 2), 32) * 32) * 16.0 * cin * N;
        return 2.0 * B * H * W * 9.0 * cin * N;
    };
    auto res = [&](const ResW& r, int H, int W, int c0, int c1, bool fast) {
        if (fast) {
            f += 2.0 * B * H * W * (2.0 * ((9 * r.ci + 1) / 2)) * r.co;
            f += 2.0 * B * H * W * (double)r.ci * r.co;
        } else {
            f += conv3(r.c1, H, W, c0, c1, r.co, true);
            if (r.has_res) f += conv_flops(DDK_CONV1X1, B, H, W, c0 + c1, r.co);
        }
        f += conv3(r.c2, H, W, r.co, 0, r.co, true);
    };
    auto attn = [&](const AttnW& a, int H, int W) {
        if (attn_fold_eligible(*u, a, B, H, W)) {
            f += conv_flops(DDK_CONV1X1, B, H, W, a.c, 2 * HIDDEN) + 2.0 * B * HEADS * 32.0 * 32.0 * H * W;
            f += 2.0 * B * (4.0 * HIDDEN * 32.0 * a.c + (double)a.c * HIDDEN * a.c) + conv_flops(DDK_CONV1X1, B, H, W, a.c, a.c);
            return;
        }
        f += conv_flops(DDK_CONV1X1, B, H, W, a.c, 3 * HIDDEN) + conv_flops(DDK_CONV1X1, B, H, W, HIDDEN, a.c);
        f += 2.0 * 2.0 * B * HEADS * 32.0 * 32.0 * H * W;
    };
    int H = H0, W = W0, cur_c = pad32(u->cfg.in_ch);
    for (int l = 0; l < u->L; ++l) {
        const int co = u->dims[l + 1];
        res(u->down_res[2 * l], H, W, cur_c, 0, l == 0 && first_fast(*u, B, H, W));
        res(u->down_res[2 * l + 1], H, W, co, 0, false);
        attn(u->down_attn[l], H, W);
        if (l < u->L - 1) { f += conv_flops(DDK_CONV3X3_S2, B, H, W, co, co); H /= 2; W /= 2; }
        cur_c = co;
    }
    res(u->mid1, H, W, cur_c, 0, false); attn(u->mid_attn, H, W); res(u->mid2, H, W, cur_c, 0, false);
    for (int i = 0; i < u->L - 1; ++i) {
        const int lvl = u->L - 1 - i, dout = u->dims[lvl + 1], din = u->dims[lvl];
        res(u->up_res[2 * i], H, W, cur_c, dout, false);
        res(u->up_res[2 * i + 1], H, W, din, 0, false);
        attn(u->up_attn[i], H, W);
        if (u->up_conv[i].has_wu && convT_wino_use(B, H, W, din, din))
            f += 2.0 * (double)(ceil_div((long long)B * (H / 2) * (W / 2), 32) * 32) * 36.0 * din * din;
        else
            f += conv_flops(DDK_CONVT4X4_S2, B, H, W, din, din);
        H *= 2; W *= 2;
        cur_c = din;
    }
    f += conv3(u->final_conv, H, W, cur_c, 0, u->cfg.chan, true) + 2.0 * B * H * W * (double)u->cfg.chan * u->cfg.in_ch;
    return f;
}

namespace ddk {
struct SamplerLayout {
    size_t unet_floats, off_eps, off_t, off_table, off_tact_all, off_tall, total;
};
static SamplerLayout sampler_layout(const ddk_unet& u, int B, int H, int W, int t_start) {
    SamplerLayout s;
    const size_t rows = (size_t)t_start + 1;
    s.unet_floats = make_layout(u, B, H, W).total;
    s.off_eps = s.unet_floats;
    s.off_t = s.off_eps + al4((size_t)B * H * W * u.cfg.in_ch);
    s.off_table = s.off_t + al4(2 * (size_t)(B + 3));
    s.off_tact_all = s.off_table + al4(rows * u.temb_total);
    s.off_tall = s.off_tact_all + al4(rows * u.time_dim);
    s.total = s.off_tall + al4(2 * rows);
    return s;
}

__global__ void iota64_kernel(int64_t* out, int n) {
    const int i = blockIdx.x * blockDim.x + threadIdx.x;
    if (i < n) out[i] = i;
}
}


namespace ddk {
static int ensure_temb_table(ddk_unet& u, const float* P, float* ws, const SamplerLayout& sl, int t_start, int B, int H, int W,
                             hipStream_t st, const int64_t* map) {
    const int rows = t_start + 1;
    const bool same_map = map ? (u.table.map.size() == (size_t)rows && std::equal(map, map + rows, u.table.map.begin()))
                              : u.table.map.empty();
    if (u.table.ws == ws && u.table.t_start == t_start && u.table.B == B && u.table.H == H && u.table.W == W &&
        u.table.pack_epoch == u.pack_epoch && same_map)
        return DDK_OK;
    u.table.ws = nullptr;
    int64_t* t_all = reinterpret_cast<int64_t*>(ws + sl.off_tall);
    float* tact_all = ws + sl.off_tact_all;
    if (map) {
        u.table.map.assign(map, map + rows);
        DDK_HIP(hipMemcpyAsync(t_all, u.table.map.data(), (size_t)rows * sizeof(int64_t), hipMemcpyHostToDevice, st));
        DDK_HIP(hipStreamSynchronize(st));
    } else {
        u.table.map.clear();
        hipLaunchKernelGGL(iota64_kernel, dim3((unsigned)ceil_div(rows, 256)), dim3(256), 0, st, t_all, rows);
        DDK_TRY(check_launch("iota64_kernel"));
    }
    DDK_TRY(time_mlp(t_all, P + u.freqs, P + u.w1t, P + u.b1, P + u.w2t, P + u.b2, tact_all, nullptr, rows, u.time_dim, st));
    DDK_TRY(time_proj(tact_all, P + u.temb_wt, P + u.temb_bias, ws + sl.off_table, rows, u.time_dim, u.temb_total, st));
    u.table.ws = ws; u.table.t_start = t_start; u.table.B = B; u.table.H = H; u.table.W = W;
    u.table.pack_epoch = u.pack_epoch;
    return DDK_OK;
}

template <class F>
static int run_chain(ddk_unet& u, const ChainKey& key, int n_steps, bool use_graph, F&& one_step, hipStream_t st, const char* who) {
    if (!use_graph || n_steps == 1) {
        for (int k = 0; k < n_steps; ++k) DDK_TRY(one_step());
        return DDK_OK;
    }
    auto capture = [&](int steps, hipGraph_t& graph, hipGraphExec_t& exec) -> int {
        hipError_t e = hipStreamBeginCapture(st, hipStreamCaptureModeThreadLocal);
        if (e != hipSuccess) {
            set_error("%s: hipStreamBeginCapture failed (%s); the legacy NULL stream cannot be captured -- pass a created stream", who,
                      hipGetErrorString(e));
            return DDK_ERR_HIP;
// ... 289 lines not shown
```

downsampled-diffusion_amd/ddk/lib.py:

```python
import ctypes as C
import os

import torch

_HERE = os.path.dirname(os.path.abspath(__file__))
LIB_PATH = os.environ.get("DDK_LIB", os.path.join(os.path.dirname(_HERE), "csrc", "libddk.so"))


class DDKError(RuntimeError):
    pass


ABI_VERSION = 400
ERR_CLUSTER = -4


class ConvArgs(C.Structure):
    _fields_ = [
        ("kind", C.c_int), ("src0", C.c_void_p), ("src1", C.c_void_p), ("c0", C.c_int), ("c1", C.c_int),
        ("weight", C.c_void_p), ("bias", C.c_void_p), ("resid", C.c_void_p), ("out", C.c_void_p),
        ("B", C.c_int), ("H", C.c_int), ("W", C.c_int), ("N", C.c_int), ("pre_mish", C.c_int), ("post_mish", C.c_int), ("defer_reduce", C.c_int),
        ("workspace", C.c_void_p), ("workspace_bytes", C.c_size_t), ("weight_wino", C.c_void_p),
        ("gn_partials", C.c_void_p), ("gn_groups", C.c_int), ("mish_out", C.c_void_p), ("dmish_src", C.c_void_p),
    ]


class UnetConfig(C.Structure):
    _fields_ = [("in_ch", C.c_int), ("chan", C.c_int), ("n_levels", C.c_int), ("mults", C.c_int * 8)]


class SamplerArgs(C.Structure):
    _fields_ = [
        ("unet", C.c_void_p), ("packed", C.c_void_p), ("x", C.c_void_p), ("noise", C.c_void_p),
        ("c_recip", C.c_void_p), ("c_recipm1", C.c_void_p), ("c1", C.c_void_p), ("c2", C.c_void_p),
        ("sigma", C.c_void_p), ("B", C.c_int), ("H", C.c_int), ("W", C.c_int), ("t_start", C.c_int),
        ("t_end", C.c_int), ("seed", C.c_uint64), ("stream_id", C.c_uint32), ("use_graph", C.c_int),
        ("workspace", C.c_void_p), ("workspace_bytes", C.c_size_t),
    ]


class InpaintArgs(C.Structure):
    _fields_ = [
        ("timestep_map", C.POINTER(C.c_int64)), ("known", C.c_void_p), ("mask", C.c_void_p), ("ka", C.c_void_p), ("kb", C.c_void_p),
        ("ja", C.c_void_p), ("jb", C.c_void_p),
    ]


class VlbSweepArgs(C.Structure):
    _fields_ = [
        ("unet", C.c_void_p), ("packed", C.c_void_p), ("x", C.c_void_p), ("noise", C.c_void_p),
        ("sqrt_acp", C.c_void_p), ("sqrt_1m_acp", C.c_void_p), ("c_recip", C.c_void_p), ("c_recipm1", C.c_void_p),
        ("c1", C.c_void_p), ("c2", C.c_void_p), ("post_logvar", C.c_void_p), ("B", C.c_int), ("H", C.c_int), ("W", C.c_int),
        ("T", C.c_int), ("seed", C.c_uint64), ("stream_id", C.c_uint32), ("use_graph", C.c_int),
        ("workspace", C.c_void_p), ("workspace_bytes", C.c_size_t), ("vlb_t", C.c_void_p), ("l_simple_t", C.c_void_p),
    ]


class WgradReduceJob(C.Structure):
    _fields_ = [("slab", C.c_void_p), ("grad", C.c_void_p), ("bias_slab", C.c_void_p), ("grad_b", C.c_void_p), ("slab_stride", C.c_longlong),
                ("block0", C.c_longlong), ("splits", C.c_int), ("N", C.c_int), ("ntaps", C.c_int), ("cx", C.c_int), ("c_real", C.c_int),
                ("cw", C.c_int), ("c_off", C.c_int), ("reserved", C.c_int)]


class RowsSumJob(C.Structure):
    _fields_ = [("rows", C.c_void_p), ("out", C.c_void_p * 4), ("batch_stride", C.c_longlong), ("row_stride", C.c_longlong),
                ("block0", C.c_longlong), ("nbatch", C.c_int), ("nrows", C.c_int), ("n", C.c_int), ("reserved", C.c_int)]


class PackJob(C.Structure):
    _fields_ = [("src", C.c_void_p), ("dst", C.c_void_p), ("total", C.c_longlong), ("block0", C.c_longlong), ("kind", C.c_int),
                ("p", C.c_int * 7)]


_P, _I, _LL, _F, _SZ = C.c_void_p, C.c_int, C.c_longlong, C.c_float, C.c_size_t

SIGNATURES = {
    "ddk_version": (_I, []),
    "ddk_last_error": (C.c_char_p, []),
    "ddk_device_ok": (_I, []),
    "ddk_nchw_to_nhwc": (_I, [_P, _P, _I, _I, _I, _I, _I, _P]),
    "ddk_nhwc_to_nchw": (_I, [_P, _P, _I, _I, _I, _I, _I, _P]),
    "ddk_pad_channels": (_I, [_P, _P, _LL, _I, _I, _P]),
    "ddk_pack_conv_weight": (_I, [_P, _P, _I, _I, _I, _I, _I, _P]),
    "ddk_pack_convT_weight": (_I, [_P, _P, _I, _I, _P]),
    "ddk_pack_conv_weight_split": (_I, [_P, _P, _I, _I, _I, _I, _I, _I, _I, _P]),
    "ddk_pack_convT_weight_padded": (_I, [_P, _P, _I, _I, _I, _P]),
    "ddk_pack_linear_T": (_I, [_P, _P, _I, _I, _I, _I, _P]),
    "ddk_pack_conv_weight_wino": (_I, [_P, _P, _I, _I, _I, _P]),
    "ddk_pack_conv_weight_wino_dgrad": (_I, [_P, _P, _I, _I, _I, _I, _I, _P]),
    "ddk_conv_wino_splits": (_I, [_I, _I, _I, _I, _I]),
    "ddk_pack_convT_weight_wino": (_I, [_P, _P, _I, _I, _I, _P]),
    "ddk_convT_wino_splits": (_I, [_I, _I, _I, _I, _I]),
    "ddk_conv_gn_partials": (_I, [_I, _I, _I, _I, _I, _I]),
    "ddk_groupnorm_mish_partials": (_I, [_P, _P, _I, _P, _P, _P, _I, _P, _P, _I, _I, _I, _I, _F, _P]),
    "ddk_pack_conv_weight_first": (_I, [_P, _P, _I, _I, _P]),
    "ddk_conv_first_ok": (_I, [_I, _I, _I, _I, _I]),
    "ddk_conv_first": (_I, [_P, _P, _P, _P, _P, _I, _I, _I, _I, _I, _I, _P]),
    "ddk_conv1x1_ws_ok": (_I, [C.c_longlong, _I, _I]),
    "ddk_conv1x1_ws": (_I, [_P, _P, _P, _P, _P, C.c_longlong, _I, _P, _P, _F, _P]),
    "ddk_conv1x1_ws_images": (_I, [_P, _P, _P, _P, _P, C.c_longlong, _I, _P, _P, _F, _I, _P]),
    "ddk_linattn_context_kv": (_I, [_P, _P, _I, _I, _I, _P, _SZ, _P]),
    "ddk_attention_fold": (_I, [_P, _P, _P, _P, _P, _P, _P, _P, _P, _I, _I, _I, _P]),
    "ddk_groupnorm_mish_partials_res1x1": (_I, [_P, _P, _I, _P, _P, _P, _I, _P, _P, _P, _I, _P, _I, _I, _I, _I, _F, _P]),
    "ddk_final_tail": (_I, [_P, _P, _I, _P, _P, _F, _P, _P, _I, _P, _P, _P, _P, _P, _P, _P, _P, _P, C.c_uint64, C.c_uint32, _I, _I, _I, _I, _P]),
    "ddk_pack_conv_weight_local": (_I, [_P, _P, _I, _I, _I, _P]),
    "ddk_pack_conv1x1_weight_local": (_I, [_P, _P, _I, _I, _I, _P]),
    "ddk_pack_convT_weight_local": (_I, [_P, _P, _I, _I, _P]),
    "ddk_pack_conv_weight_wino_local": (_I, [_P, _P, _I, _I, _I, _P]),
    "ddk_conv3x3_gn_mish_wino_ok": (_I, [_I, _I, _I, _I, _I, _I]),
    "ddk_conv3x3_gn_mish_wino": (_I, [_P, _I, _P, _I, _P, _P, _P, _P, _P, _I, _P, _P, _I, _I, _I, _I, _I, _F, _P]),
    "ddk_conv3x3_gn_mish_slabs": (_I, [_P, _I, _LL, _P, _I, _P, _P, _P, _P, _P, _I, _P, _I, _LL, _P, _P, _I, _I, _I, _I, _I, _F, _P]),
    "ddk_attention_kv_context_workspace_bytes": (_SZ, [_I, _I]),
    "ddk_attention_kv_context_ok": (_I, [_I, _I, _I, _I]),
    "ddk_attention_kv_context": (_I, [_P, _P, _P, _P, _F, _P, _I, _I, _P, _SZ, _P]),
    "ddk_pack_qkv_operand": (_I, [_P, _P, _I, _I, _P]),
    "ddk_linattn_small_from_x": (_I, [_P, _P, _P, _P, _F, _P, _P, _I, _I, _I, _I, _P]),
    "ddk_conv3x3_gn_mish_ok": (_I, [_I, _I, _I, _I, _I, _I]),
    "ddk_conv3x3_gn_mish": (_I, [_P, _I, _P, _I, _P, _P, _P, _P, _P, _I, _P, _P, _I, _I, _I, _I, _I, _F, _P]),
    "ddk_conv_workspace_bytes": (_SZ, [_I, _I, _I, _I, _I, _I]),
    "ddk_conv_splits": (_I, [_I, _I, _I, _I, _I, _I]),
    "ddk_conv_forward": (_I, [C.POINTER(ConvArgs), _P]),
    "ddk_debug_read_stamps": (_I, [_P]),
    "ddk_groupnorm_mish": (_I, [_P, _P, _P, _P, _I, _P, _P, _I, _I, _I, _I, _F, _P, _SZ, _P]),
    "ddk_groupnorm_workspace_bytes": (_SZ, [_I, _I, _I, _I]),
    "ddk_groupnorm_mish_slabs": (_I, [_P, _I, _LL, _P, _P, _P, _P, _I, _P, _P, _I, _I, _I, _I, _F, _P]),
    "ddk_chan_layernorm": (_I, [_P, _P, _P, _P, _LL, _I, _F, _P]),
    "ddk_mish": (_I, [_P, _P, _LL, _P]),
    "ddk_tanh": (_I, [_P, _P, _LL, _P]),
    "ddk_avgpool2": (_I, [_P, _P, _I, _I, _I, _I, _P]),
    "ddk_upsample_nearest2": (_I, [_P, _P, _I, _I, _I, _I, _P]),
    "ddk_add": (_I, [_P, _P, _P, _LL, _P]),
    "ddk_linattn_context_workspace_bytes": (_SZ, [_I, _I, _I]),
    "ddk_linattn_context": (_I, [_P, _P, _I, _I, _I, _P, _SZ, _P]),
    "ddk_linattn_apply": (_I, [_P, _P, _P, _I, _I, _I, _P]),
    "ddk_linattn_fused_small": (_I, [_P, _P, _P, _I, _I, _I, _P]),
    "ddk_time_mlp": (_I, [_P, _P, _P, _P, _P, _P, _P, _P, _I, _I, _P]),
    "ddk_time_proj": (_I, [_P, _P, _P, _P, _I, _I, _I, _P]),
    "ddk_conv1x1_small_n": (_I, [_P, _P, _P, _P, _LL, _I, _I, _P]),
    "ddk_q_sample": (_I, [_P, _P, _P, _P, _P, _P, _I, _LL, _P]),
    "ddk_p_sample_update": (_I, [_P, _P, _P, _P, _P, _P, _P, _P, _P, _I, _LL, C.c_uint64, C.c_uint32, _P]),
    "ddk_p_sample_update_multistep": (_I, [_P, _P, _P, _P, _P, _P, _P, _P, _P, _I, _LL, _P]),
    "ddk_p_sample_update_inpaint": (_I, [_P] * 14 + [_I, _LL, C.c_uint64, C.c_uint32, _P]),
    "ddk_randn": (_I, [_P, _LL, C.c_uint64, C.c_uint32, C.c_uint32, _P]),
    "ddk_fix_samples": (_I, [_P, _P, _I, _I, _I, _I, _P]),
    "ddk_sq_err_sum": (_I, [_P, _P, _P, _I, _LL, _P]),
    "ddk_vlb_terms_workspace_bytes": (_SZ, [_I, _LL]),
    "ddk_vlb_terms": (_I, [_P, _P, _P, _P, _P, _P, _P, _P, _P, _P, _P, _P, _I, _LL, _P, _SZ, _P]),
    "ddk_unet_create": (_P, [C.POINTER(UnetConfig)]),
    "ddk_unet_destroy": (None, [_P]),
    "ddk_unet_num_slots": (_I, [_P]),
    "ddk_unet_slot_name": (C.c_char_p, [_P, _I]),
    "ddk_unet_slot_numel": (_LL, [_P, _I]),
    "ddk_unet_packed_bytes": (_SZ, [_P]),
    "ddk_unet_pack_slot": (_I, [_P, _I, _P, _P, _P]),
    "ddk_unet_finalize_pack": (_I, [_P, _P, _P]),
    "ddk_unet_workspace_bytes": (_SZ, [_P, _I, _I, _I]),
    "ddk_unet_forward": (_I, [_P, _P, _P, _P, _P, _I, _I, _I, _P, _SZ, _P]),
    "ddk_conv3x3_gn_mish_cluster_ok": (_I, [_I, _I, _I, _I, _I, _I]),
    "ddk_conv3x3_gn_mish_cluster_workspace_bytes": (_SZ, [_I, _I, _I, _I]),
    "ddk_conv3x3_gn_mish_cluster_split_workspace_bytes": (_SZ, [_I, _I, _I, _I, _I, _I]),
    "ddk_conv3x3_gn_mish_cluster": (_I, [_P, _I, _P, _I, _P, _P, _P, _P, _P, _I, _P, _P, _I, _I, _I, _I, _I, _F, _P, _SZ, _P]),
    "ddk_unet_set_option": (_I, [_P, _I, _I]),
    "ddk_debug_cluster_timeouts": (C.c_uint, []),
    "ddk_conv3x3_gn_mish_cluster_check": (_I, [_P, _I, _P]),
    "ddk_unet_cluster_check": (_I, [_P, _P, _I, _I, _I, _P]),
    "ddk_debug_occupy": (_I, [_I, _I, _I, _P]),
    "ddk_debug_clock_probe": (_I, [_P, _I, _P]),
    "ddk_unet_flops": (C.c_double, [_P, _I, _I, _I]),
    "ddk_unet_flops_executed": (C.c_double, [_P, _I, _I, _I]),
    "ddk_sampler_workspace_bytes": (_SZ, [_P, _I, _I, _I, _I]),
    "ddk_sampler_run": (_I, [C.POINTER(SamplerArgs), _P]),
    "ddk_sampler_run_spaced": (_I, [C.POINTER(SamplerArgs), C.POINTER(C.c_int64), _P]),
    "ddk_sampler_multistep_workspace_bytes": (_SZ, [_P, _I, _I, _I, _I]),
    "ddk_sampler_run_multistep": (_I, [C.POINTER(SamplerArgs), C.POINTER(C.c_int64), _P, _P]),
    "ddk_sampler_inpaint_workspace_bytes": (_SZ, [_P, _I, _I, _I, _I]),
# ... 100 lines not shown
```

downsampled-diffusion_amd/ddk/ops.py:

```python
import ctypes as C

import torch

from . import lib as L

CONV3X3_S1, CONV3X3_S2, CONV1X1, CONVT4X4_S2 = 0, 1, 2, 3
GN_GROUPS, GN_EPS, LN_EPS = 8, 1e-5, 1e-5


def pad32(c):
    return (c + 31) // 32 * 32


class _PackEntry:
    __slots__ = ("wref", "out", "job", "fresh", "pooled")


_pack_cache = {}
_weights_epoch = [0]
_pack_table = {}
pack_stats = {"single": 0, "batched_launches": 0, "batched_jobs": 0}
_graph_tables = []
_graph_keep = [_graph_tables]

# ... 85 lines not shown
def cached_pack(tag, w, fn):
    import weakref
    key = (tag, w.data_ptr(), tuple(w.shape))
    e = _pack_cache.get(key)
    if e is not None and e.wref() is w:
        if e.fresh == _state(w):
            return e.out
        if e.job is not None and w.is_contiguous() and _repack_stale() and e.fresh == _state(w):
            return e.out
    e = _PackEntry()
    e.wref, e.out, e.fresh = weakref.ref(w), fn(w.detach()), _state(w)
    e.job = _pack_job(tag, w) if w.is_contiguous() and w.dtype == torch.float32 else None
    e.pooled = bool(w.is_cuda and torch.cuda.is_current_stream_capturing())
    pack_stats["single"] += 1
    _pack_table.clear()
    _pack_cache[key] = e
    return e.out


def _f32(t):
    if t.dtype != torch.float32:
        raise L.DDKError(f"expected float32, got {t.dtype}")
    return t


def nchw_to_nhwc(x, c_pad=None):
    b, c, h, w = x.shape
    c_pad = c if c_pad is None else c_pad
    out = torch.empty((b, h, w, c_pad), device=x.device, dtype=torch.float32)
    L.check(L.load().ddk_nchw_to_nhwc(L.ptr(_f32(x)), L.ptr(out), b, c, h, w, c_pad, L.stream()), "nchw_to_nhwc")
    return out


def nhwc_to_nchw(x, c=None):
    b, h, w, cs = x.shape
    c = cs if c is None else c
    out = torch.empty((b, c, h, w), device=x.device, dtype=torch.float32)
    L.check(L.load().ddk_nhwc_to_nchw(L.ptr(_f32(x)), L.ptr(out), b, c, h, w, cs, L.stream()), "nhwc_to_nchw")
    return out


def pad_channels(x, c_pad):
    c = x.shape[-1]
    out = torch.empty((*x.shape[:-1], c_pad), device=x.device, dtype=torch.float32)
    L.check(L.load().ddk_pad_channels(L.ptr(_f32(x)), L.ptr(out), x.numel() // c, c, c_pad, L.stream()), "pad_channels")
    return out


def pack_conv_weight(w):
    o, i, kh, kw = w.shape
    out = torch.empty((o, kh * kw, pad32(i)), device=w.device, dtype=torch.float32)
    L.check(L.load().ddk_pack_conv_weight(L.ptr(_f32(w.contiguous())), L.ptr(out), o, i, kh, kw, pad32(i), L.stream()),
            "pack_conv_weight")
    return out


def pack_convT_weight(w):
    i, o, kh, kw = w.shape
    if (kh, kw) != (4, 4):
        raise L.DDKError("pack_convT_weight: kernel must be 4x4")
    out = torch.empty((4, o, 4, i), device=w.device, dtype=torch.float32)
    L.check(L.load().ddk_pack_convT_weight(L.ptr(_f32(w.contiguous())), L.ptr(out), i, o, L.stream()), "pack_convT_weight")
    return out


def pack_conv_weight_wino(w):
    o, i, kh, kw = w.shape
    if (kh, kw) != (3, 3):
        raise L.DDKError("pack_conv_weight_wino: kernel must be 3x3")
    out = torch.empty((pad32(i) // 32, 16, o, 32), device=w.device, dtype=torch.float32)
    L.check(L.load().ddk_pack_conv_weight_wino(L.ptr(_f32(w.contiguous())), L.ptr(out), o, i, pad32(i), L.stream()), "pack_conv_weight_wino")
    return out


def pack_convT_weight_wino(w):
    i, o, kh, kw = w.shape
    if (kh, kw) != (4, 4):
        raise L.DDKError("pack_convT_weight_wino: kernel must be 4x4")
    out = torch.empty((4, pad32(i) // 32, 9, o, 32), device=w.device, dtype=torch.float32)
    L.check(L.load().ddk_pack_convT_weight_wino(L.ptr(_f32(w.contiguous())), L.ptr(out), i, o, pad32(i), L.stream()), "pack_convT_weight_wino")
    return out


def pack_conv_weight_local(w):
    o, i, kh, kw = w.shape
    if (kh, kw) != (3, 3) or o % 32:
        raise L.DDKError("pack_conv_weight_local: kernel must be 3x3 and O % 32 == 0")
    out = torch.empty((o // 32, 9, pad32(i) // 32, 1024), device=w.device, dtype=torch.float32)
    L.check(L.load().ddk_pack_conv_weight_local(L.ptr(_f32(w.contiguous())), L.ptr(out), o, i, pad32(i), L.stream()), "pack_conv_weight_local")
    return out


def pack_conv_weight_wino_local(w):
    o, i, kh, kw = w.shape
    if (kh, kw) != (3, 3) or o % 32:
        raise L.DDKError("pack_conv_weight_wino_local: kernel must be 3x3 and O % 32 == 0")
    out = torch.empty((o // 32, pad32(i) // 32, 16, 1024), device=w.device, dtype=torch.float32)
    L.check(L.load().ddk_pack_conv_weight_wino_local(L.ptr(_f32(w.contiguous())), L.ptr(out), o, i, pad32(i), L.stream()),
            "pack_conv_weight_wino_local")
    return out


def wino_weight(weight, x_shape, c_lo=None, c_hi=None, dgrad=False):
    b, h, w_, cin_x = x_shape
    o, i = weight.shape[0], weight.shape[1]
    if tuple(weight.shape[2:]) != (3, 3):
        return None
    if dgrad:
        lo, hi = (0 if c_lo is None else c_lo), (i if c_hi is None else c_hi)
        n_out, cin = hi - lo, o
    else:
        lo, hi, n_out, cin = 0, i, o, pad32(i)
    if L.load().ddk_conv_wino_splits(b, h, w_, pad32(cin), n_out) <= 0:
        return None
    if dgrad:
        def pack(t):
            out = torch.empty((pad32(o) // 32, 16, hi - lo, 32), device=t.device, dtype=torch.float32)
            L.check(L.load().ddk_pack_conv_weight_wino_dgrad(L.ptr(_f32(t.contiguous())), L.ptr(out), o, i, lo, hi, pad32(o), L.stream()),
                    "pack_conv_weight_wino_dgrad")
            return out
        return cached_pack(("wino_dgrad", lo, hi), weight, pack)
    return cached_pack("wino", weight, pack_conv_weight_wino)


def conv(kind, x, w_packed, bias=None, n_out=None, x2=None, resid=None, pre_mish=False, post_mish=False, w_wino=None, mish_out=None,
         dmish_src=None, leave_slabs=False):
    b, h, w_, c0 = x.shape
    c1 = 0 if x2 is None else x2.shape[-1]
    n = n_out if n_out is not None else (w_packed.shape[1] if kind == CONVT4X4_S2 else w_packed.shape[0])
    if kind == CONV3X3_S2:
        ho, wo = (h - 1) // 2 + 1, (w_ - 1) // 2 + 1
    elif kind == CONVT4X4_S2:
        ho, wo = 2 * h, 2 * w_
    elif kind == 4:
        ho, wo = h // 2, w_ // 2
    else:
        ho, wo = h, w_
    out = torch.empty((b, ho, wo, n), device=x.device, dtype=torch.float32)
    lib = L.load()
    ws_bytes = lib.ddk_conv_workspace_bytes(kind, b, h, w_, c0 + c1, n)
    if mish_out is not None or dmish_src is not None:
        w_wino = None
    wsplits = 0
    if w_wino is not None and kind == CONV3X3_S1 and not pre_mish:
        wsplits = lib.ddk_conv_wino_splits(b, h, w_, c0 + c1, n)
        if wsplits > 0:
            ws_bytes = wsplits * out.numel() * 4 if wsplits > 1 else 0
    nslab = 1
    if leave_slabs:
        if resid is not None or pre_mish or post_mish or mish_out is not None or dmish_src is not None:
            raise L.DDKError("conv(leave_slabs): only for a plain conv (bias is the consumer's to add)")
        nslab = wsplits if (w_wino is not None and kind == CONV3X3_S1 and wsplits > 0) else lib.ddk_conv_splits(kind, b, h, w_, c0 + c1, n)
        if nslab > 1 and ws_bytes < nslab * out.numel() * 4:
            raise L.DDKError("conv(leave_slabs): internal: workspace smaller than the slabs")
    ws = torch.empty(max(ws_bytes, 16) // 4, device=x.device, dtype=torch.float32) if ws_bytes else None
    a = L.ConvArgs(kind, L.ptr(_f32(x)), L.ptr(x2), c0, c1, L.ptr(w_packed), L.ptr(bias), L.ptr(resid), L.ptr(out),
                   b, h, w_, n, int(pre_mish), int(post_mish), int(leave_slabs and nslab > 1), L.ptr(ws), ws_bytes, L.ptr(w_wino), None, 0,
                   L.ptr(mish_out), L.ptr(dmish_src))
    L.check(lib.ddk_conv_forward(C.byref(a), L.stream()), "conv_forward")
    if leave_slabs:
        return out, (ws[:nslab * out.numel()].view(nslab, b, ho, wo, n) if nslab > 1 else None)
    return out


def conv_with_gn_partials(x, w_packed, bias, w_wino, x2=None, groups=GN_GROUPS):
    b, h, w_, c0 = x.shape
# ... 935 lines not shown
```

downsampled-diffusion_amd/ddk/plan.py:

```python
import ctypes as C
import math
import warnings

import torch

from . import lib as L


def sinusoidal_freqs(dim):
    half = dim // 2
    step = math.log(10000) / (half - 1)
    return torch.exp(torch.arange(half) * -step)


SAMPLERS = {"smp": ("sample", "sampler", "sampler"), "sms": ("sample_multistep", "sampler_multistep", "multistep sampler"),
            "sin": ("sample_inpaint", "sampler_inpaint", "inpainting sampler")}
CHAIN_WORKSPACES = (*SAMPLERS, "vsw")


class UnetPlan:
    def __init__(self, in_ch, chan, mults):
        lib = L.load()
        cfg = L.UnetConfig(in_ch, chan, len(mults), (C.c_int * 8)(*list(mults) + [0] * (8 - len(mults))))
        self._lib = lib
        self.handle = lib.ddk_unet_create(C.byref(cfg))
        if not self.handle:
            raise L.DDKError(f"ddk_unet_create failed: {L.last_error()}")
        self.in_ch, self.chan, self.mults = in_ch, chan, tuple(mults)
        self.slot_names = [lib.ddk_unet_slot_name(self.handle, i).decode() for i in range(lib.ddk_unet_num_slots(self.handle))]
        self.slot_numel = [lib.ddk_unet_slot_numel(self.handle, i) for i in range(len(self.slot_names))]
        self.packed = None
        self._ws = {}
        self._state = {}
        self._cluster = 1
        self._cluster_dev = None

    def __deepcopy__(self, memo):
        return None

    def __del__(self):
        try:
            if getattr(self, "handle", None):
                self._lib.ddk_unet_destroy(self.handle)
                self.handle = None
        except Exception:
            pass

    def pack(self, tensors, device):
        lib = self._lib
        nbytes = lib.ddk_unet_packed_bytes(self.handle)
        packed = torch.zeros(nbytes // 4, device=device, dtype=torch.float32)
        keep = []
        for i, name in enumerate(self.slot_names):
            if name == "@sinusoidal_freqs":
                src = sinusoidal_freqs(self.chan)
            else:
                if name not in tensors:
                    raise L.DDKError(f"UNet weight '{name}' missing from the state dict")
                src = tensors[name]
            src = src.detach().to(device=device, dtype=torch.float32).contiguous()
            if src.numel() != self.slot_numel[i]:
                raise L.DDKError(f"UNet weight '{name}': expected {self.slot_numel[i]} elements, got {src.numel()}")
            keep.append(src)
            L.check(lib.ddk_unet_pack_slot(self.handle, i, L.ptr(src), L.ptr(packed), L.stream()), f"pack {name}")
        torch.cuda.current_stream().synchronize()
        self.packed = packed
        return packed

    def _workspace(self, kind, nbytes, device):
        key = (kind, nbytes, str(device))
        hit = self._ws.get(key)
        if hit is not None:
            self._ws[key] = self._ws.pop(key)
            return hit
        if kind in CHAIN_WORKSPACES:
            mine = [k for k in self._ws if k[0] == kind]
            if len(mine) >= 3:
                old = self._ws[mine[0]]
                L.check(self._lib.ddk_sampler_release_workspace(self.handle, L.ptr(old)), "sampler_release_workspace")
                del self._ws[mine[0]]
        else:
            for k in [k for k in self._ws if k[0] == kind]:
                del self._ws[k]
        buf = torch.empty(max(nbytes, 16) // 4 + 4, device=device, dtype=torch.float32)
        self._ws[key] = buf
        return buf

    OPT_CLUSTER_GROUPNORM = 1
    OPT_ATTENTION_FOLD = 3
    OPT_FOLD_DOWNSAMPLE_REDUCE = 5
    OPT_ATTENTION_KV_CONTEXT = 6
    OPT_LEVEL_CHAIN = 7
    OPT_FIRST_GROUPNORM = 8

    def set_option(self, option, value):
        L.check(self._lib.ddk_unet_set_option(self.handle, option, int(value)), "unet_set_option")
        if option == self.OPT_CLUSTER_GROUPNORM:
            self._cluster = max(0, min(2, int(value)))

    def _cluster_failed(self, ws, b, h, w, stream_ptr):
        rc = self._lib.ddk_unet_cluster_check(self.handle, L.ptr(ws), b, h, w, stream_ptr)
        if rc == 0:
            return False
        if rc != L.ERR_CLUSTER:
            L.check(rc, "unet_cluster_check")
        warnings.warn("ddk: " + L.last_error() + " -- switching DDK_OPT_CLUSTER_GROUPNORM off for this plan and rerunning",
                      RuntimeWarning, stacklevel=3)
        self.set_option(self.OPT_CLUSTER_GROUPNORM, 0)
        return True

    def _chain_guarded(self):
        if self._cluster_dev is None:
            self._cluster_dev = self._lib.ddk_conv3x3_gn_mish_cluster_ok(32, 32, 32, 128, 128, 8) > 0
        return self._cluster >= 1 and self._cluster_dev

    def _run_chain(self, who, call, ws, b, h, w, graphed, restore=None):
        guard = self._chain_guarded()
        for rerun in (False, True):
            if rerun and restore is not None:
                restore()
            if graphed:
                cur = torch.cuda.current_stream()
                side = _side_stream(ws.device)
                side.wait_stream(cur)
                with torch.cuda.stream(side):
                    call(side.cuda_stream)
                    failed = guard and self._cluster >= 1 and self._cluster_failed(ws, b, h, w, side.cuda_stream)
                cur.wait_stream(side)
            else:
                call(L.stream())
                failed = guard and self._cluster >= 1 and self._cluster_failed(ws, b, h, w, L.stream())
            if not failed:
                return
        raise L.DDKError(f"{who}: in-launch GroupNorm reported a failure with the option off")

    def cluster_timeouts(self):
        return int(self._lib.ddk_debug_cluster_timeouts())

    def flops(self, b, h, w):
        return self._lib.ddk_unet_flops(self.handle, b, h, w)

    def flops_executed(self, b, h, w):
        return self._lib.ddk_unet_flops_executed(self.handle, b, h, w)

    def forward_nhwc(self, x, t):
        if self.packed is None:
            raise L.DDKError("UnetPlan.forward before pack()")
        b, h, w, c = x.shape
        if c != self.in_ch:
            raise L.DDKError(f"expected {self.in_ch} input channels, got {c}")
        if t.dtype != torch.int64:
            raise L.DDKError("timesteps must be int64")
        lib = self._lib
        nbytes = lib.ddk_unet_workspace_bytes(self.handle, b, h, w)
        if nbytes == 0:
            raise L.DDKError(f"unet workspace query failed: {L.last_error()}")
        ws = self._workspace("fwd", nbytes, x.device)
        out = torch.empty_like(x)
        for _ in range(2):
            L.check(lib.ddk_unet_forward(self.handle, L.ptr(self.packed), L.ptr(x), L.ptr(t), L.ptr(out), b, h, w,
                                         L.ptr(ws), nbytes, L.stream()), "unet_forward")
            if self._cluster < 2 or not self._cluster_failed(ws, b, h, w, L.stream()):
                break
        return out

    def _need_packed(self, kind):
        if self.packed is None:
            raise L.DDKError(f"UnetPlan.{SAMPLERS[kind][0]} before pack()")

    def _run_sampler(self, kind, x, t_start, t_end, bytes_query, call, use_graph):
        _, who, label = SAMPLERS[kind]
        b, h, w, _ = x.shape
        nbytes = bytes_query(b, h, w)
        if nbytes == 0:
            raise L.DDKError(f"{label} workspace query failed: {L.last_error()}")
        ws = self._workspace(kind, nbytes, x.device)
# ... 129 lines not shown
```

include/ddk.h:

```cpp
#ifndef DDK_H
#define DDK_H

#include <stddef.h>
#include <stdint.h>

#ifdef __cplusplus
extern "C" {
#endif

typedef void* ddk_stream_t;

#define DDK_OK 0
#define DDK_ERR_ARG (-1)
#define DDK_ERR_HIP (-2)
#define DDK_ERR_WORKSPACE (-3)
#define DDK_ERR_CLUSTER (-4)

int ddk_version(void);
const char* ddk_last_error(void);
int ddk_device_ok(void);

int ddk_nchw_to_nhwc(const float* src, float* dst, int B, int C, int H, int W, int c_pad, ddk_stream_t s);
int ddk_nhwc_to_nchw(const float* src, float* dst, int B, int C, int H, int W, int c_stride, ddk_stream_t s);
int ddk_pad_channels(const float* src, float* dst, long long M, int C, int c_pad, ddk_stream_t s);
// ... 93 lines not shown
int ddk_chan_layernorm(const float* x, const float* g, const float* b, float* out, long long M, int C,
                       float eps, ddk_stream_t s);
int ddk_mish(const float* x, float* out, long long n, ddk_stream_t s);
int ddk_tanh(const float* x, float* out, long long n, ddk_stream_t s);
int ddk_avgpool2(const float* x, float* out, int B, int H, int W, int C, ddk_stream_t s);
int ddk_upsample_nearest2(const float* x, float* out, int B, int H, int W, int C, ddk_stream_t s);
int ddk_add(const float* a, const float* b, float* out, long long n, ddk_stream_t s);

size_t ddk_linattn_context_workspace_bytes(int B, int HW, int heads);
int ddk_linattn_context(const float* qkv, float* ctx, int B, int HW, int heads, void* workspace, size_t workspace_bytes, ddk_stream_t s);
int ddk_linattn_context_kv(const float* kv, float* ctx, int B, int HW, int heads, void* workspace, size_t workspace_bytes, ddk_stream_t s);
int ddk_attention_fold(const float* ctx, const float* wqg, const float* c1q, const float* c2q, const float* wout, const float* bout, float* A,
                       float* a1, float* a2, int B, int C, int heads, ddk_stream_t s);
size_t ddk_attention_kv_context_workspace_bytes(int B, int HW);
int ddk_attention_kv_context_ok(int B, int HW, int C, int heads);
int ddk_attention_kv_context(const float* x, const float* w_kv, const float* c1, const float* c2, float ln_eps, float* ctx, int B, int HW,
                             void* workspace, size_t workspace_bytes, ddk_stream_t s);
int ddk_linattn_fused_small(const float* qkv, float* ctx, float* out, int B, int HW, int heads, ddk_stream_t s);
int ddk_linattn_apply(const float* qkv, const float* ctx, float* out, int B, int HW, int heads, ddk_stream_t s);
int ddk_pack_qkv_operand(const float* folded_w, float* dst, int heads, int c_pad, ddk_stream_t s);
int ddk_linattn_small_from_x(const float* x, const float* w_operand, const float* c1, const float* c2, float ln_eps, float* ctx,
                             float* out, int B, int HW, int C, int heads, ddk_stream_t s);

int ddk_time_mlp(const int64_t* t, const float* freqs, const float* w1t, const float* b1, const float* w2t,
                 const float* b2, float* act, float* raw, int B, int dim, ddk_stream_t s);
int ddk_time_proj(const float* act, const float* wt, const float* bias, float* out, int B, int dim, int n_out,
                  ddk_stream_t s);

int ddk_conv1x1_small_n(const float* x, const float* w, const float* bias, float* out, long long M, int C,
                        int n_out, ddk_stream_t s);

int ddk_q_sample(const float* x, const float* eps, const int64_t* t, const float* sqrt_acp,
                 const float* sqrt_1m_acp, float* out, int B, long long per, ddk_stream_t s);
int ddk_p_sample_update(float* x, const float* eps_hat, const float* noise, const int64_t* t,
                        const float* c_recip, const float* c_recipm1, const float* c1, const float* c2,
                        const float* sigma, int B, long long per, uint64_t seed, uint32_t stream_id,
                        ddk_stream_t s);
int ddk_p_sample_update_multistep(float* x, const float* eps_hat, float* x0_hist, const int64_t* t, const float* c_recip,
                                  const float* c_recipm1, const float* c1, const float* c2, const float* c3, int B, long long per,
                                  ddk_stream_t s);
int ddk_p_sample_update_inpaint(float* x, const float* eps_hat, const float* known, const float* mask, const int64_t* t,
                                const float* c_recip, const float* c_recipm1, const float* c1, const float* c2, const float* sigma,
                                const float* ka, const float* kb, const float* ja, const float* jb, int B, long long per, uint64_t seed,
                                uint32_t stream_id, ddk_stream_t s);
int ddk_final_tail(const float* raw, const float* partials, int tiles_per_image, const float* gamma, const float* beta, float eps,
                   const float* w, const float* bias, int n_out, float* eps_out, float* x, const float* noise, const int64_t* t,
                   const float* c_recip, const float* c_recipm1, const float* c1, const float* c2, const float* sigma, uint64_t seed,
                   uint32_t stream_id, int B, int HW, int C, int groups, ddk_stream_t s);
int ddk_randn(float* out, long long n, uint64_t seed, uint32_t step, uint32_t stream_id, ddk_stream_t s);
int ddk_fix_samples(const float* x_nchw, float* out_nhwc, int B, int C, int H, int W, ddk_stream_t s);
size_t ddk_vlb_terms_workspace_bytes(int B, long long per);
int ddk_vlb_terms(const float* x, const float* x_t, const float* eps_hat, const float* eps, const int64_t* t,
                  const float* c_recip, const float* c_recipm1, const float* c1, const float* c2,
                  const float* post_logvar, float* vlb, float* sqerr, int B, long long per, void* workspace,
                  size_t workspace_bytes, ddk_stream_t s);
int ddk_sq_err_sum(const float* a, const float* b, float* per_sample, int B, long long per, ddk_stream_t s);

typedef struct ddk_unet_config {
    int in_ch;
    int chan;
    int n_levels;
    int mults[8];
} ddk_unet_config;

typedef struct ddk_unet ddk_unet;

ddk_unet* ddk_unet_create(const ddk_unet_config* cfg);
void ddk_unet_destroy(ddk_unet* u);
int ddk_unet_num_slots(const ddk_unet* u);
const char* ddk_unet_slot_name(const ddk_unet* u, int slot);
long long ddk_unet_slot_numel(const ddk_unet* u, int slot);
size_t ddk_unet_packed_bytes(const ddk_unet* u);
int ddk_unet_pack_slot(const ddk_unet* u, int slot, const float* canonical, void* packed, ddk_stream_t s);
int ddk_unet_finalize_pack(const ddk_unet* u, void* packed, ddk_stream_t s);
size_t ddk_unet_workspace_bytes(const ddk_unet* u, int B, int H, int W);
int ddk_unet_forward(const ddk_unet* u, const void* packed, const float* x, const int64_t* t, float* out,
                     int B, int H, int W, void* workspace, size_t workspace_bytes, ddk_stream_t s);
#define DDK_OPT_CLUSTER_GROUPNORM 1
#define DDK_OPT_ATTENTION_FOLD 3
#define DDK_OPT_FOLD_DOWNSAMPLE_REDUCE 5
#define DDK_OPT_ATTENTION_KV_CONTEXT 6
#define DDK_OPT_LEVEL_CHAIN 7
#define DDK_OPT_FIRST_GROUPNORM 8
int ddk_unet_set_option(ddk_unet* u, int option, int value);
int ddk_unet_cluster_check(const ddk_unet* u, void* workspace, int B, int H, int W, ddk_stream_t s);
unsigned ddk_debug_cluster_timeouts(void);
int ddk_debug_clock_probe(unsigned long long* out, int workgroups, ddk_stream_t s);
int ddk_debug_occupy(int workgroups, int lds_bytes, int microseconds, ddk_stream_t s);
double ddk_unet_flops(const ddk_unet* u, int B, int H, int W);
double ddk_unet_flops_executed(const ddk_unet* u, int B, int H, int W);

typedef struct ddk_sampler_args {
    const ddk_unet* unet;
    const void* packed;
    float* x;
    const float* noise;
    const float* c_recip;
    const float* c_recipm1;
    const float* c1;
    const float* c2;
    const float* sigma;
    int B, H, W;
    int t_start;
    int t_end;
    uint64_t seed;
    uint32_t stream_id;
    int use_graph;
    void* workspace;
    size_t workspace_bytes;
} ddk_sampler_args;

size_t ddk_sampler_workspace_bytes(const ddk_unet* u, int B, int H, int W, int t_start);
int ddk_sampler_run(const ddk_sampler_args* a, ddk_stream_t s);
int ddk_sampler_run_spaced(const ddk_sampler_args* a, const int64_t* timestep_map, ddk_stream_t s);
size_t ddk_sampler_multistep_workspace_bytes(const ddk_unet* u, int B, int H, int W, int t_start);
int ddk_sampler_run_multistep(const ddk_sampler_args* a, const int64_t* timestep_map, const float* c3, ddk_stream_t s);
typedef struct ddk_inpaint_args {
    const int64_t* timestep_map;
    const float* known;
    const float* mask;
    const float* ka;
    const float* kb;
    const float* ja;
    const float* jb;
} ddk_inpaint_args;
size_t ddk_sampler_inpaint_workspace_bytes(const ddk_unet* u, int B, int H, int W, int n_ops);
int ddk_sampler_run_inpaint(const ddk_sampler_args* a, const ddk_inpaint_args* ip, ddk_stream_t s);
int ddk_sampler_invalidate(ddk_unet* u);
int ddk_sampler_release_workspace(ddk_unet* u, const void* workspace);

typedef struct ddk_vlb_sweep_args {
    const ddk_unet* unet;
    const void* packed;
    const float* x;
    const float* noise;
    const float* sqrt_acp;
    const float* sqrt_1m_acp;
    const float* c_recip;
    const float* c_recipm1;
    const float* c1;
    const float* c2;
    const float* post_logvar;
    int B, H, W;
    int T;
    uint64_t seed;
    uint32_t stream_id;
    int use_graph;
    void* workspace;
    size_t workspace_bytes;
    float* vlb_t;
    float* l_simple_t;
} ddk_vlb_sweep_args;

size_t ddk_vlb_sweep_workspace_bytes(const ddk_unet* u, int B, int H, int W, int T);
int ddk_vlb_sweep_run(const ddk_vlb_sweep_args* a, ddk_stream_t s);



int ddk_pack_conv_weight_wino_dgrad(const float* w_oihw, float* dst, int O, int I, int c_lo, int c_hi, int o_pad, ddk_stream_t s);
int ddk_pack_convT_weight_wino(const float* w_iohw, float* dst, int I, int O, int i_pad, ddk_stream_t s);
int ddk_convT_wino_splits(int B, int H, int W, int cin, int N);
int ddk_pack_conv_weight_dgrad(const float* w_oihw, float* dst, int O, int I, int KH, int KW, int i_pad, int o_pad,
                               ddk_stream_t s);
int ddk_zero_stuff2(const float* in, float* out, int B, int H, int W, int Ho, int Wo, int C, ddk_stream_t s);
size_t ddk_conv_wgrad_workspace_bytes(int kind, int B, int H, int W, int cx, int N);
int ddk_conv_wgrad(int kind, const float* x, const float* dy, float* grad_w, int B, int H, int W, int cx, int c_real,
                   int cw, int c_off, int N, void* workspace, size_t workspace_bytes, ddk_stream_t s);
int ddk_conv_wgrad_bias(int kind, const float* x, const float* dy, float* grad_w, float* grad_b, int B, int H, int W, int cx, int c_real,
                        int cw, int c_off, int N, void* workspace, size_t workspace_bytes, ddk_stream_t s);
int ddk_bias_grad(const float* dy, float* grad_b, long long M, int N, int accumulate, void* workspace,
                  size_t workspace_bytes, ddk_stream_t s);
size_t ddk_groupnorm_train_workspace_bytes(int B, int HW, int C, int groups);
int ddk_dropout_epoch(unsigned long long set_to, int bump, ddk_stream_t s);
int ddk_groupnorm_mish_train_fwd(const float* x, const float* gamma, const float* beta, const float* temb,
                                 int temb_stride, const float* addend, float drop_p, uint64_t seed, uint32_t layer,
                                 float* out, int B, int HW, int C, int groups, float eps, void* workspace,
                                 size_t workspace_bytes, ddk_stream_t s);
int ddk_groupnorm_mish_bwd(const float* x, const float* gamma, const float* beta, float drop_p, uint64_t seed,
                           uint32_t layer, const float* dy, float* dx, float* part, int B, int HW, int C, int groups,
                           float eps, void* workspace, size_t workspace_bytes, ddk_stream_t s);
int ddk_groupnorm_mish_train_fwd_slabs(const float* slabs, int nslab, long long slab_stride, const float* conv_bias, float* raw_out,
                                       const float* gamma, const float* beta, const float* temb, int temb_stride,
                                       const float* addend, float drop_p, uint64_t seed, uint32_t layer, float* out, int B, int HW,
                                       int C, int groups, float eps, ddk_stream_t s);
int ddk_groupnorm_mish_bwd_slabs(const float* x, const float* gamma, const float* beta, float drop_p, uint64_t seed, uint32_t layer,
                                 const float* dy_slabs, int nslab, long long slab_stride, float* dx, float* part, int B, int HW,
                                 int C, int groups, float eps, ddk_stream_t s);
int ddk_rows_sum(const float* rows, int nrows, long long row_stride, float* out, int n, int accumulate, ddk_stream_t s);
int ddk_rows_sum_batched(const float* rows, int nbatch, long long batch_stride, int nrows, long long row_stride, float* out,
                         int n, int accumulate, ddk_stream_t s);
int ddk_rows_sum_targets(const float* rows, int nbatch, long long batch_stride, int nrows, long long row_stride, float* out0, float* out1,
                         float* out2, float* out3, int n, int accumulate, ddk_stream_t s);
typedef struct ddk_rows_sum_job {
    const float* rows;
    float* out[4];
    long long batch_stride, row_stride;
    long long block0;
    int nbatch, nrows, n, reserved;
} ddk_rows_sum_job;
int ddk_rows_sum_jobs(const ddk_rows_sum_job* jobs_host, int n, ddk_stream_t s);
int ddk_multi_add(const float* src, const long long* table, int nseg, long long max_count, ddk_stream_t s);
enum {
    DDK_PACK_CONV = 0,
    DDK_PACK_CONVT = 1,
    DDK_PACK_DGRAD = 2,
    DDK_PACK_WINO = 3,
    DDK_PACK_WINO_DGRAD = 4
};
typedef struct ddk_pack_job {
    const float* src;
    float* dst;
    long long total;
    long long block0;
    int kind;
    int p[7];
} ddk_pack_job;
typedef struct ddk_wgrad_reduce_job {
    const float* slab;
    float* grad;
    const float* bias_slab;
    float* grad_b;
    long long slab_stride;
    long long block0;
    int splits, N, ntaps, cx, c_real, cw, c_off, reserved;
} ddk_wgrad_reduce_job;

int ddk_groupnorm_mish_generic_train_fwd(const float* x, const float* gamma, const float* beta, const float* temb, int temb_stride,
                                         const float* addend, float drop_p, unsigned long long seed, unsigned layer, float* out, int B, int HW,
                                         int CP, int C, int groups, float eps, ddk_stream_t s);
int ddk_groupnorm_mish_generic_bwd(const float* x, const float* gamma, const float* beta, float drop_p, unsigned long long seed, unsigned layer,
                                   const float* dy, float* dx, float* part, int B, int HW, int CP, int C, int groups, float eps,
                                   ddk_stream_t s);
int ddk_chan_layernorm_generic(const float* x, const float* g, const float* b, float* out, long long M, int CP, int C, float eps,
                               ddk_stream_t s);
int ddk_chan_layernorm_generic_bwd(const float* x, const float* g, const float* dy, const float* addend, float* dx, float* part,
                                   int max_parts, int* nparts_out, long long M, int CP, int C, float eps, ddk_stream_t s);
int ddk_conv_wgrad_defer(int kind, const float* x, const float* dy, float* grad_w, float* grad_b, int B, int H, int W, int cx, int c_real,
                         int cw, int c_off, int N, void* workspace, size_t workspace_bytes, ddk_wgrad_reduce_job* job_out, ddk_stream_t s);
int ddk_wgrad_reduce_jobs(const ddk_wgrad_reduce_job* jobs_host, int n, ddk_stream_t s);
long long ddk_pack_jobs_layout(ddk_pack_job* jobs_host, int n);
int ddk_pack_jobs(const ddk_pack_job* jobs_dev, int n, long long blocks, ddk_stream_t s);
int ddk_chan_layernorm_bwd(const float* x, const float* g, const float* dy, float* dx, float* part, int max_parts,
                           int* nparts_out, long long M, int C, float eps, ddk_stream_t s);
int ddk_chan_layernorm_bwd_add(const float* x, const float* g, const float* dy, const float* addend, float* dx, float* part,
// ... 34 lines not shown
```

Measured before the change: 26.08.

## Add polyphase Winograd kernel for stride-2 downsample convolutions

Adds a Winograd F(2x2,3x3) kernel for the stride-2 3x3 downsample convolutions. It splits the input into four polyphase components, which gives 25 non-zero transformed weight blocks instead of 36 direct multiplies per output quad. Weights are pre-packed into the new layout, and the UNet forward routes downsample convs through it when the workgroup count is at least 192. Input loads are double-buffered through a producer/consumer warp split into LDS. The aim is to cut the MFMA work of the strided convs, at the cost of an extra weight copy and a separate code path that may not fill the GPU on small shapes.

Result: no change. 26.20, median of 6 (+0.5%).

```diff
diff --git a/downsampled-diffusion_amd/csrc/conv_wino.hip b/downsampled-diffusion_amd/csrc/conv_wino.hip
--- a/downsampled-diffusion_amd/csrc/conv_wino.hip
+++ b/downsampled-diffusion_amd/csrc/conv_wino.hip
@@ -497,6 +497,7 @@
 
 #include "conv_wino2_kernel.inc"
 #include "conv_winoT_kernel.inc"
+#include "conv_winoD_kernel.inc"
 
 enum { WINO_V_OLD = 0, WINO_V_D = 1, WINO_V_F = 2 };
 static int wino_variant(int B, int H, int W, int N) {
@@ -570,7 +571,51 @@
     return check_launch("convT_wino_kernel");
 }
 
+static long long conv_s2_wino_wgs(int B, int H, int W, int N) {
+    return ceil_div((long long)B * ((H / 2 + 1) / 2) * ((W / 2 + 1) / 2), WBT) * (N / WD_NT);
+}
+bool conv_s2_wino_ok(int B, int H, int W, int cin, int N) {
+    if (B <= 0 || H < 2 || W < 2 || H % 2 || W % 2 || cin <= 0 || cin % 32 || N <= 0 || N % WD_NT) return false;
+    if ((long long)B * H * W * cin * 4 >= (1LL << 31) || (long long)B * (H / 2) * (W / 2) * N * 4 >= (1LL << 31)) return false;
+    return conv_s2_wino_wgs(B, H, W, N) < (1LL << 16);
+}
+bool conv_s2_wino_pays(int B, int H, int W, int cin, int N) {
+    return conv_s2_wino_ok(B, H, W, cin, N) && conv_s2_wino_wgs(B, H, W, N) >= 192;
+}
+int conv_s2_wino_forward(const float* x, const float* wu, const float* bias, float* out, int B, int H, int W, int cin, int N, hipStream_t st) {
+    DDK_REQUIRE(x && wu && out && aligned16(x) && aligned16(wu) && aligned16(bias) && aligned16(out), "conv_s2_wino: pointers (16-byte aligned)");
+    DDK_REQUIRE(conv_s2_wino_ok(B, H, W, cin, N), "conv_s2_wino: shape not eligible (ddk_conv_s2_wino_ok)");
+    DDK_TRY(ensure_device_init());
+    WinoDParams p{};
+    p.src = x; p.wu = wu; p.bias = bias; p.out = out;
+    p.c0 = cin; p.B = B; p.H = H; p.W = W; p.Ho = H / 2; p.Wo = W / 2; p.TH = (p.Ho + 1) / 2; p.TW = (p.Wo + 1) / 2;
+    p.N = N; p.tiles = B * p.TH * p.TW; p.chunks = cin / 32;
+    p.dTW = make_fastdiv_u((unsigned)p.TW);
+    p.dTH = make_fastdiv_u((unsigned)p.TH);
+#ifdef DDK_HOST_SANITIZE
+    san::extent("conv_s2_wino src", x, (long long)B * H * W * cin * 4);
+    san::extent("conv_s2_wino filter", wu, (long long)WD_BLOCKS * N * cin * 4);
+    san::extent("conv_s2_wino bias", bias, (long long)N * 4);
+    san::extent("conv_s2_wino out", out, (long long)B * p.Ho * p.Wo * N * 4);
+#endif
+    dim3 grid((unsigned)ceil_div(p.tiles, WBT), (unsigned)(N / WD_NT));
+#ifdef DDK_TUNING
+    if (getenv("DDK_WINO_STAMPS")) {
+        hipLaunchKernelGGL(conv_s2_wino_kernel<1>, grid, dim3(512), WD_LDS_FL * sizeof(float), st, p);
+        return check_launch("conv_s2_wino_kernel<dbg>");
+    }
+#endif
+    hipLaunchKernelGGL(conv_s2_wino_kernel<0>, grid, dim3(512), WD_LDS_FL * sizeof(float), st, p);
+    return check_launch("conv_s2_wino_kernel");
+}
+
 int conv_wino_init_device() {
+    DDK_HIP(hipFuncSetAttribute(reinterpret_cast<const void*>(&conv_s2_wino_kernel<0>), hipFuncAttributeMaxDynamicSharedMemorySize,
+                                (int)(WD_LDS_FL * sizeof(float))));
+#ifdef DDK_TUNING
+    DDK_HIP(hipFuncSetAttribute(reinterpret_cast<const void*>(&conv_s2_wino_kernel<1>), hipFuncAttributeMaxDynamicSharedMemorySize,
+                                (int)(WD_LDS_FL * sizeof(float))));
+#endif
     DDK_HIP(hipFuncSetAttribute(reinterpret_cast<const void*>(&convT_wino_kernel<0>), hipFuncAttributeMaxDynamicSharedMemorySize,
                                 (int)(WT_LDS_FL * sizeof(float))));
 #ifdef DDK_TUNING
@@ -797,6 +842,32 @@
                        I, O, i_pad, total);
     return check_launch("pack_convT_weight_wino_kernel");
 }
+extern "C" int ddk_pack_conv_s2_weight_wino(const float* w_oihw, float* dst, int O, int I, int i_pad, ddk_stream_t s) {
+    using namespace ddk;
+    DDK_REQUIRE(w_oihw && dst && O > 0 && O % WD_NT == 0 && I > 0 && i_pad >= I && i_pad % 32 == 0,
+                "pack_conv_s2_weight_wino: arguments (O % 32 == 0, i_pad % 32 == 0)");
+    const long long total = (long long)O * i_pad;
+    DDK_REQUIRE(total < (1LL << 31), "pack_conv_s2_weight_wino: 2^31 (n, c) pairs or more");
+    const long long blocks = ceil_div(total, 256);
+    hipLaunchKernelGGL(pack_conv_s2_weight_wino_kernel, dim3((unsigned)(blocks < 4096 ? blocks : 4096)), dim3(256), 0, as_stream(s), w_oihw,
+                       dst, O, I, i_pad, total);
+    return check_launch("pack_conv_s2_weight_wino_kernel");
+}
+extern "C" int ddk_conv_s2_wino_ok(int B, int H, int W, int cin, int N) { return ddk::conv_s2_wino_ok(B, H, W, cin, N) ? 1 : 0; }
+extern "C" int ddk_conv_s2_wino_block(int block, int* phase, int* position) {
+    if (block < 0 || block >= ddk::WD_BLOCKS || !phase || !position) return DDK_ERR_ARG;
+    int ph = 3;
+    while (block < ddk::wd_blk0(ph)) --ph;
+    const int k = block - ddk::wd_blk0(ph), nj = 3 - ddk::wd_j0(ph);
+    *phase = ph;
+    *position = (ddk::wd_i0(ph) + k / nj) * 3 + ddk::wd_j0(ph) + k % nj;
+    return DDK_OK;
+}
+extern "C" int ddk_conv_s2_wino(const float* x, const float* weight_wino, const float* bias, float* out, int B, int H, int W, int cin, int N,
+                                ddk_stream_t s) {
+    return ddk::conv_s2_wino_forward(x, weight_wino, bias, out, B, H, W, cin, N, ddk::as_stream(s));
+}
+
 extern "C" int ddk_convT_wino_splits(int B, int H, int W, int cin, int N) {
     if (!ddk::convT_wino_ok(H, W, cin, N)) return 0;
     return ddk::convT_wino_splits(B, H, W, cin, N);
diff --git a/downsampled-diffusion_amd/csrc/conv_winoD_kernel.inc b/downsampled-diffusion_amd/csrc/conv_winoD_kernel.inc
--- /dev/null
+++ b/downsampled-diffusion_amd/csrc/conv_winoD_kernel.inc
@@ -0,0 +1,263 @@
+
+constexpr int WD_NT = 32;
+constexpr int WD_BLOCKS = 25;
+constexpr int WD_IMG = WBT * 32;
+constexpr int WD_V_FL = 9 * WD_IMG;
+constexpr int WD_STAGE = 2 * WD_V_FL;
+constexpr int WD_LDS_FL = 2 * WD_STAGE;
+constexpr int WD_TP = WD_NT + 4;
+static_assert(4 * 4 * WBT * WD_TP <= WD_LDS_FL, "epilogue staging fits");
+
+__host__ __device__ constexpr int wd_i0(int ph) { return (ph >> 1) ? 0 : 1; }
+__host__ __device__ constexpr int wd_j0(int ph) { return (ph & 1) ? 0 : 1; }
+__host__ __device__ constexpr int wd_nblk(int ph) { return (3 - wd_i0(ph)) * (3 - wd_j0(ph)); }
+__host__ __device__ constexpr int wd_blk0(int ph) { return ph == 0 ? 0 : wd_blk0(ph - 1) + wd_nblk(ph - 1); }
+static_assert(wd_blk0(3) + wd_nblk(3) == WD_BLOCKS, "25 non-zero (position, phase) blocks");
+
+struct WinoDParams {
+    const float* src;
+    const float* wu;
+    const float* bias;
+    float* out;
+    int c0, B, H, W, Ho, Wo, TH, TW;
+    int N, tiles, chunks;
+    FastDivU dTW, dTH;
+};
+
+__global__ __launch_bounds__(256) void pack_conv_s2_weight_wino_kernel(const float* __restrict__ w, float* __restrict__ dst, int O, int I,
+                                                                       int i_pad, long long total) {
+    for (long long idx = blockIdx.x * 256LL + threadIdx.x; idx < total; idx += (long long)gridDim.x * 256) {
+        const int c = (int)(idx % i_pad);
+        const int o = (int)(idx / i_pad);
+        float k[3][3];
+#pragma unroll
+        for (int a = 0; a < 3; ++a)
+#pragma unroll
+            for (int b = 0; b < 3; ++b) k[a][b] = c < I ? w[(((long long)o * I + c) * 3 + a) * 3 + b] : 0.f;
+        const long long chunks = i_pad / 32;
+        float* base = dst + ((((long long)(o >> 5)) * chunks + (c >> 5)) * WD_BLOCKS) * WD_IMG + (o & 31) * 32 + (c & 31);
+#pragma unroll
+        for (int ph = 0; ph < 4; ++ph) {
+            const int a = ph >> 1, b = ph & 1;
+            float t[3][3];
+#pragma unroll
+            for (int kx = 0; kx < 3; ++kx) {
+                t[0][kx] = a ? k[0][kx] : 0.f;
+                t[1][kx] = a ? k[0][kx] + k[2][kx] : k[1][kx];
+                t[2][kx] = a ? k[2][kx] : k[1][kx];
+            }
+            int blk = wd_blk0(ph);
+#pragma unroll
+            for (int i = 0; i < 3; ++i) {
+                const float u[3] = {b ? t[i][0] : 0.f, b ? t[i][0] + t[i][2] : t[i][1], b ? t[i][2] : t[i][1]};
+#pragma unroll
+                for (int j = 0; j < 3; ++j)
+                    if (i >= wd_i0(ph) && j >= wd_j0(ph)) base[(long long)(blk++) * WD_IMG] = u[j];
+            }
+        }
+    }
+}
+
+template <int DBG>
+__global__ __launch_bounds__(512) void conv_s2_wino_kernel(const WinoDParams p) {
+    extern __shared__ __attribute__((aligned(16))) float smem[];
+    unsigned long long r_entry = 0;
+    if (DBG) r_entry = __builtin_amdgcn_s_memrealtime();
+    const int tid = threadIdx.x, lane = tid & 63;
+    const int wid = __builtin_amdgcn_readfirstlane(tid >> 6);
+    int tile_m, tile_n;
+    {
+        const int nwg = gridDim.x * gridDim.y;
+        const int bid = blockIdx.x + gridDim.x * blockIdx.y;
+        const int q = nwg >> 3, r = nwg & 7, xcd = bid & 7, idx = bid >> 3;
+        const int logical = (xcd < r ? xcd * (q + 1) : r * (q + 1) + (xcd - r) * q) + idx;
+        tile_n = logical % gridDim.y;
+        tile_m = logical / gridDim.y;
+    }
+    const int t0 = tile_m * WBT, n0 = tile_n * WD_NT;
+    const int n_chunks = p.chunks;
+    const int n_stages = n_chunks * 4;
+    const unsigned lds_base = (unsigned)(size_t)(__attribute__((address_space(3))) float*)smem;
+
+    if (wid >= 4) {
+        const int lw = wid - 4;
+        const int lt = lw * 64 + lane;
+        const int t = lt >> 3, cq = lt & 7;
+        __builtin_amdgcn_s_setprio(3);
+        const int g = t0 + t;
+        const bool tile_ok = g < p.tiles;
+        const unsigned gg = tile_ok ? (unsigned)g : 0u;
+        const unsigned tmp = fdiv_u(gg, p.dTW);
+        const int tx = (int)(gg - tmp * (unsigned)p.TW);
+        const unsigned bq = fdiv_u(tmp, p.dTH);
+        const int ty = (int)(tmp - bq * (unsigned)p.TH), b = (int)bq;
+        const int y0 = 4 * ty - 1, x0 = 4 * tx - 1;
+        const int pix0 = (b * p.H + y0) * p.W + x0;
+        const i32x4 srd = make_srd(p.src, (unsigned)((long long)p.B * p.H * p.W * p.c0 * 4));
+        unsigned voff[25];
+#pragma unroll
+        for (int py = 0; py < 5; ++py)
+#pragma unroll
+            for (int px = 0; px < 5; ++px) {
+                const bool ok = tile_ok && (unsigned)(y0 + py) < (unsigned)p.H && (unsigned)(x0 + px) < (unsigned)p.W;
+                voff[py * 5 + px] = ok ? (unsigned)(((pix0 + py * p.W + px) * p.c0 + cq * 4) * 4) : WINO_OOB;
+            }
+        const int v_off = t * 32 + ((cq ^ ((t >> 1) & 7)) << 2);
+        const int prow = lane >> 3, ppos = lane & 7;
+        const unsigned u_voff = (unsigned)((prow * 32 + ((ppos ^ (((lw & 1) << 2) + (prow >> 1))) << 2)) * 4);
+        const float* u_tile = p.wu + ((long long)tile_n * n_chunks * WD_BLOCKS) * WD_IMG + lw * 256;
+        auto load_phase = [&](f32x4 (&q)[9], auto phc, int chunk) {
+            constexpr int ph = decltype(phc)::value;
+            const unsigned soff = (unsigned)(chunk * 32 * 4);
+#pragma unroll
+            for (int dy = wd_i0(ph); dy < 3; ++dy)
+#pragma unroll
+                for (int dx = wd_j0(ph); dx < 3; ++dx)
+                    buf_load16(q[dy * 3 + dx], voff[(2 * dy + (ph >> 1) - 1) * 5 + 2 * dx + (ph & 1) - 1], srd, soff);
+        };
+        auto pin = [&](f32x4 (&q)[9]) {
+#pragma unroll
+            for (int i = 0; i < 9; ++i) asm volatile("" : "+v"(q[i]));
+        };
+        auto issue_u = [&](auto phc, int chunk, int buf) {
+            constexpr int ph = decltype(phc)::value;
+            const float* base = u_tile + ((long long)chunk * WD_BLOCKS + wd_blk0(ph)) * WD_IMG;
+            const unsigned dst = lds_base + (unsigned)((buf * WD_STAGE + WD_V_FL + lw * 256) * 4);
+#pragma unroll
+            for (int k = 0; k < wd_nblk(ph); ++k) lds_dma16_s(base + k * WD_IMG, u_voff, dst + (unsigned)(k * WD_IMG * 4));
+        };
+        auto write_v = [&](const f32x4 (&q)[9], auto phc, int buf) {
+            constexpr int ph = decltype(phc)::value;
+            float* base = smem + buf * WD_STAGE + v_off;
+            int k = 0;
+#pragma unroll
+            for (int i = wd_i0(ph); i < 3; ++i)
+#pragma unroll
+                for (int j = wd_j0(ph); j < 3; ++j, ++k) {
+                    f32x4 cj[3];
+#pragma unroll
+                    for (int r = (i == 0 ? 0 : 1); r < (i == 2 ? 3 : 2); ++r)
+                        cj[r] = j == 0 ? q[r * 3 + 0] - q[r * 3 + 1] : j == 1 ? q[r * 3 + 1] : q[r * 3 + 1] - q[r * 3 + 2];
+                    *reinterpret_cast<f32x4*>(base + k * WD_IMG) = i == 0 ? cj[0] - cj[1] : i == 1 ? cj[1] : cj[1] - cj[2];
+                }
+        };
+        f32x4 qa[9], qb[9];
+        load_phase(qa, std::integral_constant<int, 0>{}, 0);
+        load_phase(qb, std::integral_constant<int, 1>{}, 0);
+        issue_u(std::integral_constant<int, 0>{}, 0, 0);
+        wait_vmcnt<wd_nblk(1) + wd_nblk(0)>();
+        pin(qa);
+        write_v(qa, std::integral_constant<int, 0>{}, 0);
+        wait_vmcnt<0>();
+        asm volatile("s_waitcnt lgkmcnt(0)" ::: "memory");
+        __builtin_amdgcn_s_barrier();
+        for (int c = 0; c < n_chunks; ++c) {
+            static_for<4>([&](auto phc) {
+                constexpr int ph = decltype(phc)::value;
+                const int S = c * 4 + ph;
+                if (S + 2 < n_stages) {
+                    if constexpr ((ph & 1) == 0) load_phase(qa, std::integral_constant<int, (ph + 2) & 3>{}, c + (ph >= 2 ? 1 : 0));
+                    else load_phase(qb, std::integral_constant<int, (ph + 2) & 3>{}, c + (ph >= 2 ? 1 : 0));
+                }
+                if (S + 1 < n_stages) {
+                    issue_u(std::integral_constant<int, (ph + 1) & 3>{}, c + (ph == 3 ? 1 : 0), (ph + 1) & 1);
+                    if constexpr ((ph & 1) == 0) { pin(qb); write_v(qb, std::integral_constant<int, (ph + 1) & 3>{}, (ph + 1) & 1); }
+                    else { pin(qa); write_v(qa, std::integral_constant<int, (ph + 1) & 3>{}, (ph + 1) & 1); }
+                }
+                wait_vmcnt<0>();
+                asm volatile("s_waitcnt lgkmcnt(0)" ::: "memory");
+                __builtin_amdgcn_s_barrier();
+            });
+        }
+    } else {
+        f32x16 acc[9];
+#pragma unroll
+        for (int q = 0; q < 9; ++q)
+#pragma unroll
+            for (int r = 0; r < 16; ++r) acc[q][r] = 0.f;
+        const int fsw = ((lane & 31) >> 1) & 7, fh = lane >> 5;
+        const int foff = (lane & 31) * 32 + (((2 * wid + fh) ^ fsw) << 2);
+        __builtin_amdgcn_s_barrier();
+        unsigned long long r_loop0 = 0;
+        if (DBG) r_loop0 = __builtin_amdgcn_s_memrealtime();
+        auto mma4 = [&](f32x16& c, const float4& av, const float4& bv) {
+            c = __builtin_amdgcn_mfma_f32_32x32x2f32(av.x, bv.x, c, 0, 0, 0);
+            c = __builtin_amdgcn_mfma_f32_32x32x2f32(av.y, bv.y, c, 0, 0, 0);
+            c = __builtin_amdgcn_mfma_f32_32x32x2f32(av.z, bv.z, c, 0, 0, 0);
+            c = __builtin_amdgcn_mfma_f32_32x32x2f32(av.w, bv.w, c, 0, 0, 0);
+        };
+        for (int c = 0; c < n_chunks; ++c) {
+            static_for<4>([&](auto phc) {
+                constexpr int ph = decltype(phc)::value;
+                constexpr int nj = 3 - wd_j0(ph), nb = wd_nblk(ph);
+                const float* As = smem + (ph & 1) * WD_STAGE + foff;
+                const float* Bs = As + WD_V_FL;
+                float4 a[2], b[2];
+                a[0] = *reinterpret_cast<const float4*>(As);
+                b[0] = *reinterpret_cast<const float4*>(Bs);
+#pragma unroll
+                for (int k = 0; k < nb; ++k) {
+                    if (k + 1 < nb) {
+                        a[(k + 1) & 1] = *reinterpret_cast<const float4*>(As + (k + 1) * WD_IMG);
+                        b[(k + 1) & 1] = *reinterpret_cast<const float4*>(Bs + (k + 1) * WD_IMG);
+                    }
+                    mma4(acc[(wd_i0(ph) + k / nj) * 3 + wd_j0(ph) + k % nj], a[k & 1], b[k & 1]);
+                }
+                __builtin_amdgcn_s_barrier();
+            });
+        }
+        if (DBG && lane == 0 && wid == 0) {
+            const int wg = (blockIdx.x + gridDim.x * blockIdx.y) & 1023;
+            g_wino_stamps[wg * 8 + 0] = r_entry;
+            g_wino_stamps[wg * 8 + 1] = r_loop0;
+            g_wino_stamps[wg * 8 + 2] = __builtin_amdgcn_s_memrealtime();
+            g_wino_stamps[wg * 8 + 3] = 0;
+            g_wino_stamps[wg * 8 + 4] = 0;
+            g_wino_stamps[wg * 8 + 5] = (unsigned long long)n_stages;
+        }
+        float* Ts = smem + wid * (4 * WBT * WD_TP);
+#pragma unroll
+        for (int r = 0; r < 16; ++r) {
+            const int row = (r & 3) + 8 * (r >> 2) + 4 * (lane >> 5);
+            float* tp = Ts + row * WD_TP + (lane & 31);
+            float tt[3][2];
+#pragma unroll
+            for (int i = 0; i < 3; ++i) {
+                tt[i][0] = acc[i * 3 + 0][r] + acc[i * 3 + 1][r];
+                tt[i][1] = acc[i * 3 + 1][r] - acc[i * 3 + 2][r];
+            }
+            tp[0 * WBT * WD_TP] = tt[0][0] + tt[1][0];
+            tp[1 * WBT * WD_TP] = tt[0][1] + tt[1][1];
+            tp[2 * WBT * WD_TP] = tt[1][0] - tt[2][0];
+            tp[3 * WBT * WD_TP] = tt[1][1] - tt[2][1];
+        }
+    }
+    __syncthreads();
+#pragma unroll
+    for (int it = 0; it < 2; ++it) {
+        const int item = tid + it * 512;
+        const int t = item >> 5, px = (item >> 3) & 3, cq = item & 7;
+        const int g = t0 + t, gn = n0 + cq * 4;
+        if (g >= p.tiles) continue;
+        const unsigned tmp = fdiv_u((unsigned)g, p.dTW);
+        const int tx = g - (int)tmp * p.TW;
+        const unsigned bq = fdiv_u(tmp, p.dTH);
+        const int ty = (int)tmp - (int)bq * p.TH;
+        const int oy = 2 * ty + (px >> 1), ox = 2 * tx + (px & 1);
+        if (oy >= p.Ho || ox >= p.Wo) continue;
+        const float* tp = smem + (px * WBT + t) * WD_TP + cq * 4;
+        const float4 q0 = *reinterpret_cast<const float4*>(tp);
+        const float4 q1 = *reinterpret_cast<const float4*>(tp + 1 * (4 * WBT * WD_TP));
+        const float4 q2 = *reinterpret_cast<const float4*>(tp + 2 * (4 * WBT * WD_TP));
+        const float4 q3 = *reinterpret_cast<const float4*>(tp + 3 * (4 * WBT * WD_TP));
+        float4 y = f4add(f4add(q0, q1), f4add(q2, q3));
+        if (p.bias) y = f4add(y, *reinterpret_cast<const float4*>(p.bias + gn));
+        *reinterpret_cast<float4*>(p.out + (((long long)bq * p.Ho + oy) * p.Wo + ox) * p.N + gn) = y;
+    }
+    if (DBG && tid == 0) {
+        asm volatile("s_waitcnt vmcnt(0)" ::: "memory");
+        const int wg = (blockIdx.x + gridDim.x * blockIdx.y) & 1023;
+        g_wino_stamps[wg * 8 + 6] = __builtin_amdgcn_s_memrealtime();
+        g_wino_stamps[wg * 8 + 7] = 1;
+    }
+}
diff --git a/downsampled-diffusion_amd/csrc/ddk_internal.h b/downsampled-diffusion_amd/csrc/ddk_internal.h
--- a/downsampled-diffusion_amd/csrc/ddk_internal.h
+++ b/downsampled-diffusion_amd/csrc/ddk_internal.h
@@ -157,6 +157,9 @@
 bool convT_wino_ok(int H, int W, int cin, int N);
 int convT_wino_splits(int B, int H, int W, int cin, int N);
 int convT_wino_forward(const ddk_conv_args& a, int splits, hipStream_t st);
+bool conv_s2_wino_ok(int B, int H, int W, int cin, int N);
+bool conv_s2_wino_pays(int B, int H, int W, int cin, int N);
+int conv_s2_wino_forward(const float* x, const float* wu, const float* bias, float* out, int B, int H, int W, int cin, int N, hipStream_t st);
 int conv_wino_init_device();
 int conv_wino_stats_parts(int B, int H, int W, int cin, int N, int groups);
 bool conv_first_ok(int cin, int N, int H, int W, int groups);
diff --git a/downsampled-diffusion_amd/csrc/unet_plan.hip b/downsampled-diffusion_amd/csrc/unet_plan.hip
--- a/downsampled-diffusion_amd/csrc/unet_plan.hip
+++ b/downsampled-diffusion_amd/csrc/unet_plan.hip
@@ -17,7 +17,8 @@
 
 enum PackKind { PK_COPY = 0, PK_CONV = 1, PK_CONVT = 2, PK_LINEAR_T = 3, PK_WINO = 4, PK_LOCAL = 5, PK_WLOCAL = 6, PK_FIRST = 7, PK_CONVT_WINO = 8,
                 PK_ROWS = 9 , PK_LOCAL1 = 10 ,
-                PK_CONVT_LOCAL = 11  };
+                PK_CONVT_LOCAL = 11 ,
+                PK_S2_WINO = 12  };
 
 struct Slot {
     std::string name;
@@ -45,6 +46,8 @@
     bool has_wl1 = false;
     size_t wtl = 0;
     bool has_wtl = false;
+    size_t wd = 0;
+    bool has_wd = false;
 };
 struct NormW { size_t g = 0, b = 0; int c_real = 0; };
 struct ResW {
@@ -108,6 +111,7 @@
     bool cluster_split = true;
     bool attn_kvctx = true;
     bool fold_down_reduce = false;
+    bool down_wino = true;
     bool first_gn = true;
     int level_chain = 9;
     int level_chain_max_batch = 32;
@@ -312,7 +316,15 @@
         }
         u->down_res.push_back(u->add_res(p + "1.", co, co, cur));
         u->down_attn.push_back(u->add_attn(p + "2.", co));
-        if (l < u->L - 1) u->down_conv.push_back(u->add_conv(p + "3.conv.", co, co, 3, true, false, 0, l == u->L - 2));
+        if (l < u->L - 1) {
+            ConvW dc = u->add_conv(p + "3.conv.", co, co, 3, true, false, 0, l == u->L - 2);
+            if (!u->generic && co % 32 == 0) {
+                dc.wd = u->alloc((size_t)25 * co * co);
+                dc.has_wd = true;
+                u->slots.push_back(Slot{p + "3.conv.weight", (long long)co * co * 9, PK_S2_WINO, dc.wd, co, co, 3, 3, co, 0, 0});
+            }
+            u->down_conv.push_back(dc);
+        }
     }
     const int mid = u->dims[u->L];
     u->mid1 = u->add_res("mid_block1.", mid, mid, cur);
@@ -408,6 +420,7 @@
              p.level_chain = v == 1 ? 9 : v == 2 ? 1 : v == 3 ? 15 : v == 4 ? 6 : v == 8 ? 2 : v == 16 ? 4 : v != 0 ? 9 : 0;
          }},
         {DDK_OPT_FOLD_DOWNSAMPLE_REDUCE, true, [](ddk_unet& p, int v) { p.fold_down_reduce = v != 0; }},
+        {DDK_OPT_DOWNSAMPLE_WINO, true, [](ddk_unet& p, int v) { p.down_wino = v != 0; }},
         {10, true, [](ddk_unet& p, int v) { p.level_chain_max_batch = v; }},
         {9, true, [](ddk_unet& p, int v) { p.attn_fold_min_hw = v; }},
         {2, false, [](ddk_unet& p, int v) { p.cluster_limit = v; }},
@@ -509,6 +522,7 @@
         case PK_WLOCAL: rc = ddk_pack_conv_weight_wino_local(canonical, dst, sl.O, sl.I, sl.i_pad, s); break;
         case PK_FIRST: rc = ddk_pack_conv_weight_first(canonical, dst, sl.O, sl.I, s); break;
         case PK_CONVT_WINO: rc = ddk_pack_convT_weight_wino(canonical, dst, sl.I, sl.O, sl.i_pad, s); break;
+        case PK_S2_WINO: rc = ddk_pack_conv_s2_weight_wino(canonical, dst, sl.O, sl.I, sl.i_pad, s); break;
         default: return fail_arg("unet_pack_slot: slot kind");
     }
     DDK_TRY(rc);
@@ -535,6 +549,9 @@
 
 static bool convT_wino_use(int B, int H, int W, int cin, int N) {
     return convT_wino_ok(H, W, cin, N) && convT_wino_splits(B, H, W, cin, N) <= 2;
+}
+static bool down_wino_use(const ddk_unet& u, const ConvW& cw, int B, int H, int W, int c) {
+    return u.down_wino && cw.has_wd && conv_s2_wino_pays(B, H, W, c, c);
 }
 static bool use_wino(const ConvW& cw, int H, int W, int cin, int N) {
     return cw.has_wu && conv_wino_ok(DDK_CONV3X3_S1, H, W, cin, N);
@@ -1160,6 +1177,11 @@
         if (l < u.L - 1 && chain_edges && l + 1 == u.L - 1) {
             H /= 2; W /= 2;
             cur = skip;
+        } else if (l < u.L - 1 && down_wino_use(u, u.down_conv[l], B, H, W, co)) {
+            DDK_TRY(conv_s2_wino_forward(skip, P + u.down_conv[l].wd, u.down_conv[l].has_bias ? P + u.down_conv[l].b : nullptr, bufA, B, H, W, co,
+                                         co, st));
+            H /= 2; W /= 2;
+            cur = bufA;
         } else if (l < u.L - 1) {
             const int s2 = conv_splits(DDK_CONV3X3_S2, B, H, W, co, co);
             if (u.fold_down_reduce && s2 > 1 && !(chained && l + 1 == u.L - 1) && !(chained8 && l + 1 == u.L - 2) &&
@@ -1358,7 +1380,13 @@
         res(u->down_res[2 * l], H, W, cur_c, 0, l == 0 && first_fast(*u, B, H, W));
         res(u->down_res[2 * l + 1], H, W, co, 0, false);
         attn(u->down_attn[l], H, W);
-        if (l < u->L - 1) { f += conv_flops(DDK_CONV3X3_S2, B, H, W, co, co); H /= 2; W /= 2; }
+        if (l < u->L - 1) {
+            if (down_wino_use(*u, u->down_conv[l], B, H, W, co))
+                f += 2.0 * (double)(ceil_div((long long)B * ((H / 2 + 1) / 2) * ((W / 2 + 1) / 2), 32) * 32) * 25.0 * co * co;
+            else
+                f += conv_flops(DDK_CONV3X3_S2, B, H, W, co, co);
+            H /= 2; W /= 2;
+        }
         cur_c = co;
     }
     res(u->mid1, H, W, cur_c, 0, false); attn(u->mid_attn, H, W); res(u->mid2, H, W, cur_c, 0, false);
diff --git a/downsampled-diffusion_amd/ddk/lib.py b/downsampled-diffusion_amd/ddk/lib.py
--- a/downsampled-diffusion_amd/ddk/lib.py
+++ b/downsampled-diffusion_amd/ddk/lib.py
@@ -91,6 +91,10 @@
     "ddk_conv_wino_splits": (_I, [_I, _I, _I, _I, _I]),
     "ddk_pack_convT_weight_wino": (_I, [_P, _P, _I, _I, _I, _P]),
     "ddk_convT_wino_splits": (_I, [_I, _I, _I, _I, _I]),
+    "ddk_pack_conv_s2_weight_wino": (_I, [_P, _P, _I, _I, _I, _P]),
+    "ddk_conv_s2_wino_block": (_I, [_I, C.POINTER(_I), C.POINTER(_I)]),
+    "ddk_conv_s2_wino_ok": (_I, [_I, _I, _I, _I, _I]),
+    "ddk_conv_s2_wino": (_I, [_P, _P, _P, _P, _I, _I, _I, _I, _I, _P]),
     "ddk_conv_gn_partials": (_I, [_I, _I, _I, _I, _I, _I]),
     "ddk_groupnorm_mish_partials": (_I, [_P, _P, _I, _P, _P, _P, _I, _P, _P, _I, _I, _I, _I, _F, _P]),
     "ddk_pack_conv_weight_first": (_I, [_P, _P, _I, _I, _P]),
diff --git a/downsampled-diffusion_amd/ddk/ops.py b/downsampled-diffusion_amd/ddk/ops.py
--- a/downsampled-diffusion_amd/ddk/ops.py
+++ b/downsampled-diffusion_amd/ddk/ops.py
@@ -191,6 +191,38 @@
     return out
 
 
+def pack_conv_s2_weight_wino(w):
+    o, i, kh, kw = w.shape
+    if (kh, kw) != (3, 3) or o % 32:
+        raise L.DDKError("pack_conv_s2_weight_wino: kernel must be 3x3 and O % 32 == 0")
+    out = torch.empty((o // 32, pad32(i) // 32, 25, 32, 32), device=w.device, dtype=torch.float32)
+    L.check(L.load().ddk_pack_conv_s2_weight_wino(L.ptr(_f32(w.contiguous())), L.ptr(out), o, i, pad32(i), L.stream()),
+            "pack_conv_s2_weight_wino")
+    return out
+
+
+def conv_s2_wino_blocks():
+    out = []
+    for k in range(25):
+        ph, pos = C.c_int(), C.c_int()
+        L.check(L.load().ddk_conv_s2_wino_block(k, C.byref(ph), C.byref(pos)), "conv_s2_wino_block")
+        out.append((ph.value, pos.value))
+    return out
+
+
+def conv_s2_wino(x, w_wino, bias=None):
+    b, h, w_, c = x.shape
+    n = w_wino.shape[0] * 32
+    if w_wino.shape[1] * 32 != c:
+        raise L.DDKError(f"conv_s2_wino: filter packed for {w_wino.shape[1] * 32} input channels, input has {c}")
+    lib = L.load()
+    if not lib.ddk_conv_s2_wino_ok(b, h, w_, c, n):
+        raise L.DDKError(f"conv_s2_wino: shape {tuple(x.shape)} -> {n} not eligible")
+    out = torch.empty((b, h // 2, w_ // 2, n), device=x.device, dtype=torch.float32)
+    L.check(lib.ddk_conv_s2_wino(L.ptr(_f32(x)), L.ptr(w_wino), L.ptr(bias), L.ptr(out), b, h, w_, c, n, L.stream()), "conv_s2_wino")
+    return out
+
+
 def pack_conv_weight_local(w):
     o, i, kh, kw = w.shape
     if (kh, kw) != (3, 3) or o % 32:
diff --git a/downsampled-diffusion_amd/ddk/plan.py b/downsampled-diffusion_amd/ddk/plan.py
--- a/downsampled-diffusion_amd/ddk/plan.py
+++ b/downsampled-diffusion_amd/ddk/plan.py
@@ -92,6 +92,7 @@
     OPT_ATTENTION_KV_CONTEXT = 6
     OPT_LEVEL_CHAIN = 7
     OPT_FIRST_GROUPNORM = 8
+    OPT_DOWNSAMPLE_WINO = 12
 
     def set_option(self, option, value):
         L.check(self._lib.ddk_unet_set_option(self.handle, option, int(value)), "unet_set_option")
diff --git a/include/ddk.h b/include/ddk.h
--- a/include/ddk.h
+++ b/include/ddk.h
@@ -199,6 +199,7 @@
 #define DDK_OPT_ATTENTION_KV_CONTEXT 6
 #define DDK_OPT_LEVEL_CHAIN 7
 #define DDK_OPT_FIRST_GROUPNORM 8
+#define DDK_OPT_DOWNSAMPLE_WINO 12
 int ddk_unet_set_option(ddk_unet* u, int option, int value);
 int ddk_unet_cluster_check(const ddk_unet* u, void* workspace, int B, int H, int W, ddk_stream_t s);
 unsigned ddk_debug_cluster_timeouts(void);
@@ -277,6 +278,11 @@
 int ddk_pack_conv_weight_wino_dgrad(const float* w_oihw, float* dst, int O, int I, int c_lo, int c_hi, int o_pad, ddk_stream_t s);
 int ddk_pack_convT_weight_wino(const float* w_iohw, float* dst, int I, int O, int i_pad, ddk_stream_t s);
 int ddk_convT_wino_splits(int B, int H, int W, int cin, int N);
+int ddk_pack_conv_s2_weight_wino(const float* w_oihw, float* dst, int O, int I, int i_pad, ddk_stream_t s);
+int ddk_conv_s2_wino_block(int block, int* phase, int* position);
+int ddk_conv_s2_wino_ok(int B, int H, int W, int cin, int N);
+int ddk_conv_s2_wino(const float* x, const float* weight_wino, const float* bias, float* out, int B, int H, int W, int cin, int N,
+                     ddk_stream_t s);
 int ddk_pack_conv_weight_dgrad(const float* w_oihw, float* dst, int O, int I, int KH, int KW, int i_pad, int o_pad,
                                ddk_stream_t s);
 int ddk_zero_stuff2(const float* in, float* out, int B, int H, int W, int Ho, int Wo, int C, ddk_stream_t s);
```
